# senli1073/SeisT

Hardware: NVIDIA H100
Metric: waveforms/sec (B,3,8192) seist_m_dpk fwd+bwd (higher is better)
Workload: dtype f32

## Files before the change

seist_b200/csrc/api.cu:

```cuda
#include <atomic>
#include <cstdio>
#include <cstdlib>
#include <cstring>
#include <vector>
#include "common.cuh"

namespace seist {

static thread_local char g_err[512] = "";
static std::atomic<uint64_t> g_launches{0};
static int g_sm_count = 0;

void set_error(const char* msg) {
  std::strncpy(g_err, msg, sizeof(g_err) - 1);
  g_err[sizeof(g_err) - 1] = 0;
}
void note_launch() { g_launches.fetch_add(1, std::memory_order_relaxed); }
int check_launch(const char* what) {
  cudaError_t e = cudaPeekAtLastError();
  if (e != cudaSuccess) {
    cudaGetLastError();
    std::snprintf(g_err, sizeof(g_err), "%s: %s", what, cudaGetErrorString(e));
    return (int)e;
  }
  return 0;
}

int launch_conv_fwd(const SeistOp& op, cudaStream_t s);
int launch_conv_bwd_data(const SeistOp& op, cudaStream_t s);
int launch_conv_bwd_w(const SeistOp& op, cudaStream_t s, int sm_count);
int launch_res_bwd(const SeistOp& op, cudaStream_t s);
int launch_att_fwd(const SeistOp& op, cudaStream_t s);
int launch_att_bwd_q(const SeistOp& op, cudaStream_t s);
int launch_att_bwd_kv(const SeistOp& op, cudaStream_t s);
int launch_headvec_fwd(const SeistOp& op, cudaStream_t s);
int launch_headvec_bwd(const SeistOp& op, cudaStream_t s);
int launch_bn_finalize(const SeistOp& op, bool fwd, cudaStream_t s);
bool pw_eligible(const SeistOp& op);
int launch_pw_fwd(const SeistOp& op, cudaStream_t s, int sm_count);
int launch_pw_bwd_data(const SeistOp& op, cudaStream_t s, int sm_count);
int launch_res_bwd4(const SeistOp& op, cudaStream_t s, int sm_count);
bool bww_eligible(const SeistOp& op);
int launch_bww_any(const SeistOp& op, cudaStream_t s, int sm_count);
bool convk_eligible(const SeistOp& op);
bool bwwk_eligible(const SeistOp& op);
int launch_grad_combine(const SeistOp& op, cudaStream_t s, int sm_count);
bool convk_bwd_data_eligible(const SeistOp& op);
int launch_bwwk(const SeistOp& op, cudaStream_t s, int sm_count);
int launch_convk_fwd(const SeistOp& op, cudaStream_t s);
int launch_convk_bwd_data(const SeistOp& op, cudaStream_t s);
int launch_bn_prepare(const SeistOp& op, bool fwd, cudaStream_t s);
int launch_stem_compose(const SeistOp& op, bool fwd, cudaStream_t s);
bool tcconv_eligible(const SeistOp& op, int mode);
int launch_tcconv(const SeistOp& op, int mode, cudaStream_t s, int sm_count);
int tcconv_error_flag();

int env_knob(const char* name, int def) {
  const char* e = std::getenv(name);
  return (e && *e) ? std::atoi(e) : def;
}
int bww_waves() {
  static int v = -1;
  if (v < 0) { const char* e = std::getenv("SEIST_BWW_WAVES"); v = (e && e[0] >= '1' && e[0] <= '4') ? e[0] - '0' : 2; }
  return v;
}
static int bwwk_mode() {
  static int v = -1;
  if (v < 0) { const char* e = std::getenv("SEIST_BWWK"); v = (e && e[0] == '0') ? 0 : 1; }
  return v;
}
static int tcc_mode() {
  static int v = -1;
  if (v < 0) { const char* e = std::getenv("SEIST_TCC"); v = !e ? 2 : (e[0] == '0' ? 0 : (e[0] == '1' ? 1 : 2)); }
  return v;
}
static bool tcc_auto(const SeistOp& op, int mode) {
  const int Kd = mode == 0 ? op.Cin : op.Cout;
  if (op.up_src_L > 0) return mode == 0 && Kd >= 32;
  if (op.k > 1) return mode == 0 ? (op.L_out <= 512 && Kd >= 16) : (op.L_out <= 256 && Kd >= 32);
  return mode == 0 && Kd >= 64 && op.L_out <= 256;
}
static bool use_tcc(const SeistOp& op, int mode) {
  const int m = tcc_mode();
  if (m == 0 || !tcconv_eligible(op, mode)) return false;
  return m == 1 || tcc_auto(op, mode);
}

static int sm_count() {
  if (g_sm_count == 0) {
    int dev = 0;
    cudaGetDevice(&dev);
    if (cudaDeviceGetAttribute(&g_sm_count, cudaDevAttrMultiProcessorCount, dev) != cudaSuccess || g_sm_count <= 0)
      g_sm_count = 132;
  }
  return g_sm_count;
}

static int validate_conv(const SeistOp& op) {
  if (op.groups <= 0 || op.Cin % op.groups || op.Cout % op.groups) { set_error("conv: channels not divisible by groups"); return -2; }
  if (op.k < 1 || op.stride < 1 || op.N < 1 || op.L_out < 1) { set_error("conv: bad geometry"); return -2; }
  if (op.n_in < 1 || op.n_in > SEIST_MAX_IN) { set_error("conv: bad n_in"); return -2; }
  if ((op.pool > 1 || op.up_src_L > 0) && op.n_in != 1) { set_error("conv: pool/upsample need a single input view"); return -2; }
  if (op.pool > 1 && (op.k != 1 || op.up_src_L > 0)) { set_error("conv: pool only with k=1"); return -2; }
  if (op.N > 65535) { set_error("conv: batch > 65535 per launch"); return -2; }
  return 0;
}

enum Family {
  F_NONE = 0, F_TCCONV_FWD, F_TCCONV_BWD_DATA, F_PW_FWD, F_CONVK_FWD, F_CONV_FWD, F_PW_BWD_DATA, F_CONVK_BWD_DATA,
  F_CONV_BWD_DATA, F_BWWK, F_BWW, F_CONV_BWD_W, F_RES_BWD, F_RES_BWD4, F_ATT_FWD, F_ATT_BWD_Q, F_ATT_BWD_KV, F_HEADVEC_FWD,
  F_HEADVEC_BWD, F_BN_FINALIZE_FWD, F_BN_FINALIZE_BWD, F_BN_PREPARE_FWD, F_BN_PREPARE_BWD, F_STEM_COMPOSE_FWD, F_STEM_COMPOSE_BWD,
  F_GRAD_COMBINE, F_ZERO
};
static const char* kFamilyName[] = {
  "none", "tcconv_fwd(wgmma+TMA)", "tcconv_bwd_data(wgmma+TMA)", "pw_fwd(simt)", "convk_fwd(simt)",
  "conv_fwd(simt)", "pw_bwd_data(simt)", "convk_bwd_data(simt)", "conv_bwd_data(simt)", "bwwk(simt)", "bww(simt)",
  "conv_bwd_w(simt)", "res_bwd", "res_bwd4", "att_fwd", "att_bwd_q", "att_bwd_kv", "headvec_fwd", "headvec_bwd", "bn_finalize_fwd",
  "bn_finalize_bwd", "bn_prepare_fwd", "bn_prepare_bwd", "stem_compose_fwd", "stem_compose_bwd", "grad_combine", "zero"
};

static Family choose(const SeistOp& op) {
  switch (op.kind) {
    case SEIST_OP_CONV_FWD:
      if (use_tcc(op, 0)) return F_TCCONV_FWD;
      if (pw_eligible(op)) return F_PW_FWD;
      return convk_eligible(op) ? F_CONVK_FWD : F_CONV_FWD;
    case SEIST_OP_CONV_BWD_DATA:
      if (use_tcc(op, 1)) return F_TCCONV_BWD_DATA;
      if (pw_eligible(op)) return F_PW_BWD_DATA;
      return convk_bwd_data_eligible(op) ? F_CONVK_BWD_DATA : F_CONV_BWD_DATA;
    case SEIST_OP_CONV_BWD_W:
      if (bwwk_mode() && bwwk_eligible(op)) return F_BWWK;
      return bww_eligible(op) ? F_BWW : F_CONV_BWD_W;
    case SEIST_OP_RES_BWD: return (op.L_out & 3) ? F_RES_BWD : F_RES_BWD4;
    case SEIST_OP_ATT_FWD: return F_ATT_FWD;
    case SEIST_OP_ATT_BWD_Q: return F_ATT_BWD_Q;
    case SEIST_OP_ATT_BWD_KV: return F_ATT_BWD_KV;
    case SEIST_OP_HEADVEC_FWD: return F_HEADVEC_FWD;
    case SEIST_OP_HEADVEC_BWD: return F_HEADVEC_BWD;
    case SEIST_OP_BN_FINALIZE_FWD: return F_BN_FINALIZE_FWD;
    case SEIST_OP_BN_FINALIZE_BWD: return F_BN_FINALIZE_BWD;
    case SEIST_OP_BN_PREPARE_FWD: return F_BN_PREPARE_FWD;
    case SEIST_OP_BN_PREPARE_BWD: return F_BN_PREPARE_BWD;
    case SEIST_OP_STEM_COMPOSE_FWD: return F_STEM_COMPOSE_FWD;
    case SEIST_OP_STEM_COMPOSE_BWD: return F_STEM_COMPOSE_BWD;
    case SEIST_OP_GRAD_COMBINE: return F_GRAD_COMBINE;
    case SEIST_OP_ZERO: return F_ZERO;
    default: return F_NONE;
  }
}

static int run_one(const SeistOp& op, cudaStream_t s) {
  if (op.kind == SEIST_OP_CONV_FWD || op.kind == SEIST_OP_CONV_BWD_DATA || op.kind == SEIST_OP_CONV_BWD_W) {
    int v = validate_conv(op);
    if (v) return v;
  }
  switch (choose(op)) {
    case F_TCCONV_FWD: return launch_tcconv(op, 0, s, sm_count());
    case F_TCCONV_BWD_DATA: return launch_tcconv(op, 1, s, sm_count());
    case F_PW_FWD: return launch_pw_fwd(op, s, sm_count());
    case F_CONVK_FWD: return launch_convk_fwd(op, s);
    case F_CONV_FWD: return launch_conv_fwd(op, s);
    case F_PW_BWD_DATA: return launch_pw_bwd_data(op, s, sm_count());
    case F_CONVK_BWD_DATA: return launch_convk_bwd_data(op, s);
    case F_CONV_BWD_DATA: return launch_conv_bwd_data(op, s);
    case F_BWWK: return launch_bwwk(op, s, sm_count());
    case F_BWW: return launch_bww_any(op, s, sm_count());
    case F_CONV_BWD_W: return launch_conv_bwd_w(op, s, sm_count());
    case F_RES_BWD: return launch_res_bwd(op, s);
    case F_RES_BWD4: return launch_res_bwd4(op, s, sm_count());
    case F_ATT_FWD: return launch_att_fwd(op, s);
    case F_ATT_BWD_Q: return launch_att_bwd_q(op, s);
    case F_ATT_BWD_KV: return launch_att_bwd_kv(op, s);
    case F_HEADVEC_FWD: return launch_headvec_fwd(op, s);
    case F_HEADVEC_BWD: return launch_headvec_bwd(op, s);
    case F_BN_FINALIZE_FWD: return launch_bn_finalize(op, true, s);
    case F_BN_FINALIZE_BWD: return launch_bn_finalize(op, false, s);
    case F_BN_PREPARE_FWD: return launch_bn_prepare(op, true, s);
    case F_BN_PREPARE_BWD: return launch_bn_prepare(op, false, s);
    case F_STEM_COMPOSE_FWD: return launch_stem_compose(op, true, s);
    case F_STEM_COMPOSE_BWD: return launch_stem_compose(op, false, s);
    case F_GRAD_COMBINE: return launch_grad_combine(op, s, sm_count());
    case F_ZERO: {
      cudaError_t e = cudaMemsetAsync(op.out.x, 0, op.zero_bytes, s);
      if (e != cudaSuccess) { set_error(cudaGetErrorString(e)); return (int)e; }
      return 0;
    }
    default: set_error("unknown op kind"); return -1;
  }
}

}

extern "C" {

int seist_plan_run(const SeistOp* ops, int32_t n, void* stream);
const char* seist_last_error(void);

int seist_abi_version(void) { return SEIST_ABI_VERSION; }
uint64_t seist_sizeof_op(void) { return sizeof(SeistOp); }
uint64_t seist_sizeof_bn(void) { return sizeof(SeistBN); }
const char* seist_last_error(void) { return seist::g_err; }
uint64_t seist_launch_count(void) { return seist::g_launches.load(); }
const char* seist_op_family(const SeistOp* op) { return op ? seist::kFamilyName[seist::choose(*op)] : "none"; }
int seist_tc_error_flag(void) { return seist::tcconv_error_flag(); }

static std::vector<cudaEvent_t> g_events[64];
static cudaEvent_t event_at(size_t i) {
  int dev = 0;
  cudaGetDevice(&dev);
  std::vector<cudaEvent_t>& pool = g_events[dev & 63];
  while (pool.size() <= i) {
    cudaEvent_t e = nullptr;
    if (cudaEventCreateWithFlags(&e, cudaEventDisableTiming) != cudaSuccess) return nullptr;
    pool.push_back(e);
  }
  return pool[i];
}
static int fork_join(cudaStream_t from, cudaStream_t to, size_t& ev) {
  cudaEvent_t e = event_at(ev++);
  if (e == nullptr) { seist::set_error("plan_run2: cudaEventCreate failed"); return (int)cudaErrorMemoryAllocation; }
  cudaError_t r = cudaEventRecord(e, from);
  if (r == cudaSuccess) r = cudaStreamWaitEvent(to, e, 0);
  if (r != cudaSuccess) { seist::set_error(cudaGetErrorString(r)); return (int)r; }
  return 0;
}

int seist_plan_run2(const SeistOp* ops, int32_t n, void* stream, void* side_stream) {
  if (side_stream == nullptr || side_stream == stream) return seist_plan_run(ops, n, stream);
  if (ops == nullptr || n < 0) { seist::set_error("plan_run2: bad arguments"); return -1; }
  cudaStream_t s = (cudaStream_t)stream, side = (cudaStream_t)side_stream;
  size_t ev = 0;
  bool forked = false, main_dirty = true;
  for (int i = 0; i < n; ++i) {
    const bool on_side = ops[i].kind == SEIST_OP_CONV_BWD_W || ops[i].kind == SEIST_OP_STEM_COMPOSE_BWD;
    int rc;
    if (on_side) {
      if (main_dirty) {
        const int fr = fork_join(s, side, ev);
        if (fr) return fr;
        main_dirty = false;
      }
      rc = seist::run_one(ops[i], side);
      forked = true;
    } else {
      rc = seist::run_one(ops[i], s);
      main_dirty = true;
    }
    if (rc != 0) {
      char buf[600];
      std::snprintf(buf, sizeof(buf), "op %d (kind %d): %s", i, ops[i].kind, seist::g_err);
      seist::set_error(buf);
      if (forked) fork_join(side, s, ev);
      return rc;
    }
  }
  if (forked) return fork_join(side, s, ev);
  return 0;
}

int seist_plan_run_lanes(const SeistOp* ops, int32_t n, void* const* streams, int32_t n_streams) {
  if (ops == nullptr || n < 0 || streams == nullptr || n_streams < 1 || n_streams > 8) { seist::set_error("plan_run_lanes: bad arguments"); return -1; }
  if (n_streams == 1) return seist_plan_run(ops, n, streams[0]);
  cudaStream_t s0 = (cudaStream_t)streams[0];
  size_t ev = (size_t)n;
  for (int l = 1; l < n_streams; ++l) {
    size_t e = ev;
    const int fr = fork_join(s0, (cudaStream_t)streams[l], e);
    if (fr) return fr;
  }
  int rc = 0;
  for (int i = 0; i < n && rc == 0; ++i) {
    const SeistOp& op = ops[i];
    const int lane = op.lane < 0 ? 0 : (op.lane >= n_streams ? n_streams - 1 : op.lane);
    cudaStream_t s = (cudaStream_t)streams[lane];
    for (int w = 0; w < op.n_wait && w < 4 && rc == 0; ++w) {
      if (op.wait_ev[w] < 0 || op.wait_ev[w] >= n) { seist::set_error("plan_run_lanes: bad event id"); rc = -1; break; }
      cudaEvent_t e = event_at((size_t)op.wait_ev[w]);
      cudaError_t r = e ? cudaStreamWaitEvent(s, e, 0) : cudaErrorMemoryAllocation;
      if (r != cudaSuccess) { seist::set_error(cudaGetErrorString(r)); rc = (int)r; }
    }
    if (rc) break;
    rc = seist::run_one(op, s);
    if (rc != 0) {
      char buf[600];
      std::snprintf(buf, sizeof(buf), "op %d (kind %d): %s", i, op.kind, seist_last_error());
      seist::set_error(buf);
      break;
    }
    if (op.rec_event >= 0) {
      cudaEvent_t e = op.rec_event < n ? event_at((size_t)op.rec_event) : nullptr;
      cudaError_t r = e ? cudaEventRecord(e, s) : cudaErrorMemoryAllocation;
      if (r != cudaSuccess) { seist::set_error(cudaGetErrorString(r)); rc = (int)r; }
    }
  }
  for (int l = 1; l < n_streams; ++l) {
    size_t e = (size_t)n + 1 + (size_t)l;
    const int jr = fork_join((cudaStream_t)streams[l], s0, e);
    if (jr && !rc) rc = jr;
  }
  return rc;
}

int seist_plan_run(const SeistOp* ops, int32_t n, void* stream) {
  if (ops == nullptr || n < 0) { seist::set_error("plan_run: bad arguments"); return -1; }
  cudaStream_t s = (cudaStream_t)stream;
  for (int i = 0; i < n; ++i) {
    int rc = seist::run_one(ops[i], s);
    if (rc != 0) {
      char buf[600];
      std::snprintf(buf, sizeof(buf), "op %d (kind %d): %s", i, ops[i].kind, seist::g_err);
      seist::set_error(buf);
      return rc;
    }
  }
  return 0;
}

}
```

seist_b200/csrc/tcconv.cu:

```cuda
#include <cuda.h>
#include <cstdlib>
#include <cstring>
#include "common.cuh"

namespace seist {

constexpr int TCC_EPI_WARPS = 8;
constexpr int TCC_XF_WARPS = 8;
constexpr int TCC_NT = 32 * (TCC_EPI_WARPS + TCC_XF_WARPS + 1);
constexpr int TCC_M = 128;
constexpr int TCC_MAX_STAGES = 8;
constexpr int TCC_NMAX = 128;
constexpr int TCC_ACC_PITCH = TCC_M + 4;

struct TccGeom {
  int mode;
  int Kd, Nd;
  int k, padl;
  int padA, toff;
  int src_len, dst_len;
  int KC, nchunks;
  int R, Rbox, Rp;
  int N_pad;
  int raw_stages, a_stages, b_resident;
  int n_raw;
  int raw_tensor_bytes;
  int a_part;
  int b_part;
  int a_stage;
  int has_dxd, has_bn, need_x;
  int up, up_S;
  int off_raw, off_a, off_b, off_tab_k, off_tab_n, off_red, off_acc, off_bar, smem_bytes;
};

struct TccMaps {
  CUtensorMap m[3];
};

struct TccK {
  float a, b, c;
  int view;
};
struct TccTgt {
  const float* x;
  float* g;
  long long nstride;
  float sc, sh, mu, istd;
  int act, bn, bnc, accum;
};

__device__ int g_tcc_err_dev = 0;

__device__ __forceinline__ uint32_t s32(const void* p) { return (uint32_t)__cvta_generic_to_shared(p); }

__device__ __forceinline__ uint64_t tcc_desc(uint32_t saddr, uint32_t lbo_bytes, uint32_t sbo_bytes) {
  uint64_t d = 0;
  d |= (uint64_t)((saddr >> 4) & 0x3FFFu);
  d |= (uint64_t)((lbo_bytes >> 4) & 0x3FFFu) << 16;
  d |= (uint64_t)((sbo_bytes >> 4) & 0x3FFFu) << 32;
  return d;
}
template <int N>
__device__ __forceinline__ void tcc_mma(float (&d)[N / 2], uint64_t adesc, uint64_t bdesc, uint32_t accum);
template <>
__device__ __forceinline__ void tcc_mma<32>(float (&d)[16], uint64_t adesc, uint64_t bdesc, uint32_t accum) {
  asm volatile(
      "{\n\t.reg .pred p;\n\tsetp.ne.b32 p, %18, 0;\n\t"
      "wgmma.mma_async.sync.aligned.m64n32k8.f32.tf32.tf32 {%0, %1, %2, %3, %4, %5, %6, %7, %8, %9, %10, %11, %12, %13, %14, %15}, %16, %17, p, 1, 1;\n\t}\n"
      : "+f"(d[0]), "+f"(d[1]), "+f"(d[2]), "+f"(d[3]), "+f"(d[4]), "+f"(d[5]), "+f"(d[6]), "+f"(d[7]), "+f"(d[8]), "+f"(d[9]), "+f"(d[10]), "+f"(d[11]), "+f"(d[12]), "+f"(d[13]), "+f"(d[14]), "+f"(d[15])
      : "l"(adesc), "l"(bdesc), "r"(accum));
}
template <>
__device__ __forceinline__ void tcc_mma<64>(float (&d)[32], uint64_t adesc, uint64_t bdesc, uint32_t accum) {
  asm volatile(
      "{\n\t.reg .pred p;\n\tsetp.ne.b32 p, %34, 0;\n\t"
      "wgmma.mma_async.sync.aligned.m64n64k8.f32.tf32.tf32 {%0, %1, %2, %3, %4, %5, %6, %7, %8, %9, %10, %11, %12, %13, %14, %15, %16, %17, %18, %19, %20, %21, %22, %23, %24, %25, %26, %27, %28, %29, %30, %31}, %32, %33, p, 1, 1;\n\t}\n"
      : "+f"(d[0]), "+f"(d[1]), "+f"(d[2]), "+f"(d[3]), "+f"(d[4]), "+f"(d[5]), "+f"(d[6]), "+f"(d[7]), "+f"(d[8]), "+f"(d[9]), "+f"(d[10]), "+f"(d[11]), "+f"(d[12]), "+f"(d[13]), "+f"(d[14]), "+f"(d[15]), "+f"(d[16]), "+f"(d[17]), "+f"(d[18]), "+f"(d[19]), "+f"(d[20]), "+f"(d[21]), "+f"(d[22]), "+f"(d[23]), "+f"(d[24]), "+f"(d[25]), "+f"(d[26]), "+f"(d[27]), "+f"(d[28]), "+f"(d[29]), "+f"(d[30]), "+f"(d[31])
      : "l"(adesc), "l"(bdesc), "r"(accum));
}
template <>
__device__ __forceinline__ void tcc_mma<128>(float (&d)[64], uint64_t adesc, uint64_t bdesc, uint32_t accum) {
  asm volatile(
      "{\n\t.reg .pred p;\n\tsetp.ne.b32 p, %66, 0;\n\t"
      "wgmma.mma_async.sync.aligned.m64n128k8.f32.tf32.tf32 {%0, %1, %2, %3, %4, %5, %6, %7, %8, %9, %10, %11, %12, %13, %14, %15, %16, %17, %18, %19, %20, %21, %22, %23, %24, %25, %26, %27, %28, %29, %30, %31, %32, %33, %34, %35, %36, %37, %38, %39, %40, %41, %42, %43, %44, %45, %46, %47, %48, %49, %50, %51, %52, %53, %54, %55, %56, %57, %58, %59, %60, %61, %62, %63}, %64, %65, p, 1, 1;\n\t}\n"
      : "+f"(d[0]), "+f"(d[1]), "+f"(d[2]), "+f"(d[3]), "+f"(d[4]), "+f"(d[5]), "+f"(d[6]), "+f"(d[7]), "+f"(d[8]), "+f"(d[9]), "+f"(d[10]), "+f"(d[11]), "+f"(d[12]), "+f"(d[13]), "+f"(d[14]), "+f"(d[15]), "+f"(d[16]), "+f"(d[17]), "+f"(d[18]), "+f"(d[19]), "+f"(d[20]), "+f"(d[21]), "+f"(d[22]), "+f"(d[23]), "+f"(d[24]), "+f"(d[25]), "+f"(d[26]), "+f"(d[27]), "+f"(d[28]), "+f"(d[29]), "+f"(d[30]), "+f"(d[31]), "+f"(d[32]), "+f"(d[33]), "+f"(d[34]), "+f"(d[35]), "+f"(d[36]), "+f"(d[37]), "+f"(d[38]), "+f"(d[39]), "+f"(d[40]), "+f"(d[41]), "+f"(d[42]), "+f"(d[43]), "+f"(d[44]), "+f"(d[45]), "+f"(d[46]), "+f"(d[47]), "+f"(d[48]), "+f"(d[49]), "+f"(d[50]), "+f"(d[51]), "+f"(d[52]), "+f"(d[53]), "+f"(d[54]), "+f"(d[55]), "+f"(d[56]), "+f"(d[57]), "+f"(d[58]), "+f"(d[59]), "+f"(d[60]), "+f"(d[61]), "+f"(d[62]), "+f"(d[63])
      : "l"(adesc), "l"(bdesc), "r"(accum));
}
template <int R>
__device__ __forceinline__ void tcc_keep(float (&d)[R]) {
#pragma unroll
  for (int i = 0; i < R; ++i) asm volatile("" : "+f"(d[i])::"memory");
}
__device__ __forceinline__ void tcc_arrive(uint32_t bar) {
  asm volatile("mbarrier.arrive.shared::cta.b64 _, [%0];" ::"r"(bar) : "memory");
}
__device__ __forceinline__ void tcc_expect_tx(uint32_t bar, uint32_t bytes) {
  asm volatile("mbarrier.arrive.expect_tx.shared::cta.b64 _, [%0], %1;" ::"r"(bar), "r"(bytes) : "memory");
}
__device__ __forceinline__ void tcc_tma3(uint32_t dst, const CUtensorMap* map, int c0, int c1, int c2, uint32_t bar) {
  asm volatile(
      "cp.async.bulk.tensor.3d.shared::cluster.global.tile.mbarrier::complete_tx::bytes [%0], [%1, {%2, %3, %4}], [%5];" ::"r"(dst),
      "l"((uint64_t)map), "r"(c0), "r"(c1), "r"(c2), "r"(bar)
      : "memory");
}
__device__ __forceinline__ bool tcc_wait(uint32_t bar, uint32_t parity, volatile int* abort_s) {
  uint32_t done = 0;
  for (int it = 0; it < (1 << 18); ++it) {
    asm volatile(
        "{\n\t.reg .pred p;\n\tmbarrier.try_wait.parity.shared::cta.b64 p, [%1], %2, %3;\n\tselp.b32 %0, 1, 0, p;\n\t}\n"
        : "=r"(done)
        : "r"(bar), "r"(parity), "r"(20000u)
        : "memory");
    if (done) return true;
    if ((it & 15) == 15 && *abort_s) return false;
  }
  *abort_s = 1;
  return false;
}
__device__ __forceinline__ void tcc_split(float x, float& hi, float& lo) {
  hi = __uint_as_float(__float_as_uint(x) & 0xFFFFE000u);
  lo = x - hi;
}
__device__ __forceinline__ float tcc_gelu(float x) { return gelu_f(x); }
__device__ __forceinline__ float tcc_gelu_grad(float x) { return gelu_grad_f(x); }

__device__ __forceinline__ float tcc_reduce16(float (&v)[16], int lane) {
#pragma unroll
  for (int half = 8, off = 16; half >= 1; half >>= 1, off >>= 1) {
    const bool up = (lane & off) != 0;
#pragma unroll
    for (int i = 0; i < 8; ++i) {
      if (i < half) {
        const float send = up ? v[i] : v[i + half];
        const float keep = up ? v[i + half] : v[i];
        v[i] = keep + __shfl_xor_sync(0xffffffffu, send, off);
      }
    }
  }
  return v[0] + __shfl_xor_sync(0xffffffffu, v[0], 1);
}
__device__ __forceinline__ int tcc_red_index(int lane) {
  return ((lane >> 4) & 1) * 8 + ((lane >> 3) & 1) * 4 + ((lane >> 2) & 1) * 2 + ((lane >> 1) & 1);
}

#define TCC_LD16(rr, col0)                                                                                               \
  _Pragma("unroll") for (int c_ = 0; c_ < 16; ++c_) rr[c_] = __float_as_uint(acc_s[((col0) + c_) * TCC_ACC_PITCH + srow]);

__device__ __forceinline__ int tcc_up_src0(int p0) { return ((p0 >> 1) - 1) & ~3; }

__device__ __forceinline__ float tcc_wval(const SeistOp& op, int mode, int t, int n, int c) {
  const int co = mode == 0 ? n : c, ci = mode == 0 ? c : n;
  const int tt = mode == 0 ? t : op.k - 1 - t;
  if (co >= op.Cout || ci >= op.Cin) return 0.f;
  const int cin_g = op.Cin / op.groups, cout_g = op.Cout / op.groups;
  const int g = co / cout_g;
  if (ci / cin_g != g) return 0.f;
  return __ldg(op.W + ((size_t)co * cin_g + (ci - g * cin_g)) * op.k + tt);
}

template <int MODE, bool F_GELU, bool F_ELEM, int NB>
__global__ void __launch_bounds__(TCC_NT, 1) tcconv_kernel(const __grid_constant__ SeistOp op, const __grid_constant__ TccGeom g,
                                                           const __grid_constant__ TccMaps maps) {
  extern __shared__ __align__(16) unsigned char tcc_raw[];
  unsigned char* base = tcc_raw + ((128u - (s32(tcc_raw) & 127u)) & 127u);
  unsigned char* raw_s = base + g.off_raw;
  unsigned char* a_s = base + g.off_a;
  unsigned char* b_s = base + g.off_b;
  TccK* tk_s = reinterpret_cast<TccK*>(base + g.off_tab_k);
  float* red_s = reinterpret_cast<float*>(base + g.off_red);
  uint64_t* bars = reinterpret_cast<uint64_t*>(base + g.off_bar);
  uint64_t* raw_full = bars;
  uint64_t* raw_empty = raw_full + TCC_MAX_STAGES;
  uint64_t* a_full = raw_empty + TCC_MAX_STAGES;
  uint64_t* a_empty = a_full + TCC_MAX_STAGES;
  volatile int* abort_s = reinterpret_cast<volatile int*>(a_empty + TCC_MAX_STAGES);
  float* acc_s = reinterpret_cast<float*>(base + g.off_acc);

  const int tid = threadIdx.x, lane = tid & 31;
  const int warp = __shfl_sync(0xffffffffu, tid >> 5, 0);
  const int Kd = g.Kd, Nd = g.Nd;
  const int Kd_pad = g.nchunks * g.KC;
  const int tiles_per_n = (g.dst_len + TCC_M - 1) / TCC_M;
  const int total = op.N * tiles_per_n;
  const bool has_bn_out = (op.out.bn >= 0 && op.out.g != nullptr);

  for (int c = tid; c < Kd_pad; c += TCC_NT) {
    TccK e;
    e.a = 0.f; e.b = 0.f; e.c = 0.f; e.view = 0;
    if (c < Kd) {
      if (MODE == 0) {
        int cv;
        const int vi = resolve_view(op, c, cv);
        view_coef(op, op.in[vi], cv, e.a, e.b);
        e.c = (float)op.in[vi].act;
        e.view = vi;
      } else {
        const OutGradCoef kc = out_grad_coef(op, c);
        e.a = kc.A; e.b = kc.Bx; e.c = kc.Cc;
      }
    }
    tk_s[c] = e;
  }
  if (MODE == 0) {
    float* ep_s = reinterpret_cast<float*>(base + g.off_tab_n);
    for (int co = tid; co < Nd; co += TCC_NT) {
      float b = 0.f, asc = 1.f, ash = 0.f, bsc = 1.f, bsh = 0.f;
      if (op.bias) b = op.bias[co];
      if (op.res_a.C > 0) view_coef(op, op.res_a, co, asc, ash);
      if (op.res_b.C > 0) view_coef(op, op.res_b, co, bsc, bsh);
      ep_s[co] = b;
      ep_s[Nd + co] = asc;
      ep_s[2 * Nd + co] = ash;
      ep_s[3 * Nd + co] = bsc;
      ep_s[4 * Nd + co] = bsh;
    }
  } else {
    TccTgt* tg_s = reinterpret_cast<TccTgt*>(base + g.off_tab_n);
    for (int ci = tid; ci < Nd; ci += TCC_NT) {
      int cv;
      const int vi = resolve_view(op, ci, cv);
      const SeistView& v = op.in[vi];
      TccTgt e;
      e.x = v.x + (size_t)(v.c0 + cv) * v.L;
      e.g = v.g ? v.g + (size_t)(v.c0 + cv) * v.L : nullptr;
      e.nstride = (long long)v.Ct * v.L;
      view_coef(op, v, cv, e.sc, e.sh);
      e.mu = 0.f; e.istd = 0.f;
      if (v.bn >= 0) view_khat(op, v, cv, e.mu, e.istd);
      e.act = v.act; e.bn = v.bn; e.bnc = v.bn_c0 + cv; e.accum = v.accum;
      tg_s[ci] = e;
    }
  }
  for (int i = tid; i < TCC_EPI_WARPS * 2 * Nd; i += TCC_NT) red_s[i] = 0.f;

  const int colpitchB = g.N_pad * 16;
  auto stage_b = [&](int chunk, unsigned char* b_hi, unsigned char* b_lo, int t0, int nthreads) {
    const int nq = g.KC >> 2;
    const int items = g.k * nq * g.N_pad;
    for (int idx = t0; idx < items; idx += nthreads) {
      const int n = idx % g.N_pad;
      const int rest = idx / g.N_pad;
      const int q = rest % nq, t = rest / nq;
      float4 hi, lo;
      float w[4];
#pragma unroll
      for (int j = 0; j < 4; ++j) {
        const int c = chunk * g.KC + 4 * q + j;
        w[j] = (n < Nd && c < Kd) ? tcc_wval(op, MODE, t, n, c) : 0.f;
      }
      tcc_split(w[0], hi.x, lo.x);
      tcc_split(w[1], hi.y, lo.y);
      tcc_split(w[2], hi.z, lo.z);
      tcc_split(w[3], hi.w, lo.w);
      const int off = (t * nq + q) * colpitchB + n * 16;
      *reinterpret_cast<float4*>(b_hi + off) = hi;
      *reinterpret_cast<float4*>(b_lo + off) = lo;
    }
  };
  if (g.b_resident)
    for (int ch = 0; ch < g.nchunks; ++ch) stage_b(ch, b_s + (size_t)ch * 2 * g.b_part, b_s + (size_t)ch * 2 * g.b_part + g.b_part, tid, TCC_NT);

  if (tid == 32) {
    for (int i = 0; i < TCC_MAX_STAGES; ++i) {
      asm volatile("mbarrier.init.shared::cta.b64 [%0], %1;" ::"r"(s32(&raw_full[i])), "r"(1) : "memory");
      asm volatile("mbarrier.init.shared::cta.b64 [%0], %1;" ::"r"(s32(&raw_empty[i])), "r"(TCC_XF_WARPS) : "memory");
      asm volatile("mbarrier.init.shared::cta.b64 [%0], %1;" ::"r"(s32(&a_full[i])), "r"(TCC_XF_WARPS) : "memory");
      asm volatile("mbarrier.init.shared::cta.b64 [%0], %1;" ::"r"(s32(&a_empty[i])), "r"(TCC_EPI_WARPS) : "memory");
    }
    *abort_s = 0;
    asm volatile("fence.mbarrier_init.release.cluster;" ::: "memory");
  }
  asm volatile("fence.proxy.async.shared::cta;" ::: "memory");
  __syncthreads();
  const uint64_t seed = load_seed(op.step_seed);

  if (warp == TCC_EPI_WARPS + TCC_XF_WARPS) {
    if (lane == 0) {
      int rs = 0;
      uint32_t rph = 0;
      const uint32_t stage_tx = (uint32_t)(g.n_raw * g.raw_tensor_bytes);
      const int nbox = g.KC >> 3;
      for (int tile = blockIdx.x; tile < total && !*abort_s; tile += gridDim.x) {
        const int n = tile / tiles_per_n;
        const int p0 = (tile - n * tiles_per_n) * TCC_M - g.padA;
        for (int ch = 0; ch < g.nchunks; ++ch) {
          if (!tcc_wait(s32(&raw_empty[rs]), rph ^ 1, abort_s)) break;
          const uint32_t bar = s32(&raw_full[rs]);
          tcc_expect_tx(bar, stage_tx);
          const uint32_t dst0 = s32(raw_s + (size_t)rs * g.n_raw * g.raw_tensor_bytes);
          for (int b = 0; b < nbox; ++b) {
            const int c = ch * g.KC + 8 * b;
            const uint32_t boxoff = (uint32_t)(8 * b * g.Rbox * 4);
            if (MODE == 0) {
              int cv = 0, vi = 0;
              if (c < Kd) vi = resolve_view(op, c, cv);
              else cv = 1 << 20;
              tcc_tma3(dst0 + boxoff, &maps.m[vi], g.up ? tcc_up_src0(p0) : p0, op.in[vi].c0 + cv, n, bar);
            } else {
              const int cc = c < Kd ? op.out.c0 + c : (1 << 20);
              int slot = 0;
              if (g.has_dxd) { tcc_tma3(dst0 + slot * g.raw_tensor_bytes + boxoff, &maps.m[0], p0, cc, n, bar); ++slot; }
              if (g.has_bn) { tcc_tma3(dst0 + slot * g.raw_tensor_bytes + boxoff, &maps.m[1], p0, cc, n, bar); ++slot; }
              if (g.need_x) { tcc_tma3(dst0 + slot * g.raw_tensor_bytes + boxoff, &maps.m[2], p0, cc, n, bar); ++slot; }
            }
          }
          if (++rs == g.raw_stages) { rs = 0; rph ^= 1; }
        }
      }
    }
  } else if (warp >= TCC_EPI_WARPS) {
    const int xw = warp - TCC_EPI_WARPS;
    int rs = 0, as = 0;
    uint32_t rph = 0, aph = 0;
    const int nq = g.KC >> 2, nrb = g.Rp >> 5;
    const int q = xw & (nq - 1);
    const int rb0 = xw / nq, rbs = TCC_XF_WARPS / nq;
    const int colpitchA = g.Rp * 16;
    const uint32_t thr = drop_threshold(op.p_elem);
    const float keep_s = op.p_elem > 0.f ? 1.0f / (1.0f - op.p_elem) : 1.f;
    const int raw_t = g.raw_tensor_bytes >> 2;
    for (int tile = blockIdx.x; tile < total && !*abort_s; tile += gridDim.x) {
      const int n = tile / tiles_per_n;
      const int p0 = (tile - n * tiles_per_n) * TCC_M - g.padA;
      float pfaf = 1.f;
      if (MODE == 1) pfaf = path_factor(op, seed, n) * alpha_factor(op, seed, n);
      for (int ch = 0; ch < g.nchunks; ++ch) {
        if (!tcc_wait(s32(&raw_full[rs]), rph, abort_s)) break;
        if (!tcc_wait(s32(&a_empty[as]), aph ^ 1, abort_s)) break;
        const float* raw = reinterpret_cast<const float*>(raw_s + (size_t)rs * g.n_raw * g.raw_tensor_bytes) + 4 * q * g.Rbox;
        unsigned char* a_hi = a_s + (size_t)as * g.a_stage + q * colpitchA;
        unsigned char* a_lo = a_hi + g.a_part;
        const int cbase = ch * g.KC + 4 * q;
        TccK e[4];
#pragma unroll
        for (int j = 0; j < 4; ++j) e[j] = tk_s[cbase + j];
        const int nvalid = Kd - cbase;
        for (int rb = rb0; rb < nrb; rb += 2 * rbs) {
          float t[2][4];
          int rrow[2];
          bool act[2];
#pragma unroll
          for (int h = 0; h < 2; ++h) {
            const int r = (rb + h * rbs) * 32 + lane;
            rrow[h] = r;
            act[h] = (rb + h * rbs) < nrb;
            const int p = p0 + r;
            const bool inb = act[h] && (r < g.R) && p >= 0 && p < g.src_len;
            const int rr = (act[h] && r < g.Rbox) ? r : 0;
            if (MODE == 0 && g.up) {
              const int pc = p < 0 ? 0 : p;
              const int i0 = pc == 0 ? 0 : (pc - 1) >> 1;
              const int i1 = min(i0 + 1, g.up_S - 1);
              const float w1 = pc == 0 ? 0.f : ((pc & 1) ? 0.25f : 0.75f);
              const int s0 = tcc_up_src0(p0);
              const int a0 = min(max(i0 - s0, 0), g.Rbox - 1), a1 = min(max(i1 - s0, 0), g.Rbox - 1);
#pragma unroll
              for (int j = 0; j < 4; ++j) {
                float f0 = fmaf(e[j].a, raw[j * g.Rbox + a0], e[j].b);
                float f1 = fmaf(e[j].a, raw[j * g.Rbox + a1], e[j].b);
                if (F_GELU && e[j].c != 0.f) { f0 = tcc_gelu(f0); f1 = tcc_gelu(f1); }
                const float v = fmaf(w1, f1 - f0, f0);
                t[h][j] = (inb && j < nvalid) ? v : 0.f;
              }
            } else if (MODE == 0) {
#pragma unroll
              for (int j = 0; j < 4; ++j) {
                float v = fmaf(e[j].a, raw[j * g.Rbox + rr], e[j].b);
                if (F_GELU && e[j].c != 0.f) v = tcc_gelu(v);
                t[h][j] = (inb && j < nvalid) ? v : 0.f;
              }
            } else {
              uint64_t hq = 0ull;
              if (F_ELEM) {
                const int ck = min(cbase + (lane & 3), Kd - 1);
                hq = rng_u64(seed, op.seed_elem, (((uint64_t)n * op.Cout + ck) * (uint64_t)op.L_out + (uint64_t)(inb ? p : 0)) >> 2);
              }
#pragma unroll
              for (int j = 0; j < 4; ++j) {
                const int ro = j * g.Rbox + rr;
                int slot = 0;
                float dxd = 0.f, du = 0.f, x = 0.f;
                if (g.has_dxd) { dxd = raw[ro]; ++slot; }
                if (g.has_bn) { du = raw[slot * raw_t + ro]; ++slot; }
                if (g.need_x) { x = raw[slot * raw_t + ro]; }
                float gv = dxd + fmaf(e[j].a, du, fmaf(e[j].b, x, e[j].c));
                if (op.out_act == SEIST_OUT_SIGMOID) gv *= x * (1.f - x);
                gv *= pfaf;
                if (F_ELEM) {
                  const uint64_t hh = __shfl_sync(0xffffffffu, hq, (lane & ~3) | j);
                  gv *= (((uint32_t)(hh >> (16 * (p & 3))) & 0xFFFFu) >= thr) ? keep_s : 0.f;
                }
                t[h][j] = (inb && j < nvalid) ? gv : 0.f;
              }
            }
          }
#pragma unroll
          for (int h = 0; h < 2; ++h) {
            if (!act[h]) continue;
            float4 hi, lo;
            tcc_split(t[h][0], hi.x, lo.x);
            tcc_split(t[h][1], hi.y, lo.y);
            tcc_split(t[h][2], hi.z, lo.z);
            tcc_split(t[h][3], hi.w, lo.w);
            *reinterpret_cast<float4*>(a_hi + rrow[h] * 16) = hi;
            *reinterpret_cast<float4*>(a_lo + rrow[h] * 16) = lo;
          }
        }
        if (!g.b_resident) {
          unsigned char* bst = a_s + (size_t)as * g.a_stage + 2 * g.a_part;
          stage_b(ch, bst, bst + g.b_part, xw * 32 + lane, TCC_XF_WARPS * 32);
        }
        asm volatile("fence.proxy.async.shared::cta;" ::: "memory");
        __syncwarp();
        if (lane == 0) {
          tcc_arrive(s32(&a_full[as]));
          tcc_arrive(s32(&raw_empty[rs]));
        }
        if (++rs == g.raw_stages) { rs = 0; rph ^= 1; }
        if (++as == g.a_stages) { as = 0; aph ^= 1; }
      }
    }
  } else {
    const int eg = warp >> 2, wq = warp & 3;
    const int L = g.dst_len;
    const bool stats = MODE == 0 ? ((op.out.bn >= 0) && op.bn_table[op.out.bn >= 0 ? op.out.bn : 0].use_batch) : true;
    const float* ep_s = reinterpret_cast<const float*>(base + g.off_tab_n);
    const TccTgt* tg_s = reinterpret_cast<const TccTgt*>(base + g.off_tab_n);
    const uint32_t thr = drop_threshold(op.p_elem);
    const float keep_s = op.p_elem > 0.f ? 1.0f / (1.0f - op.p_elem) : 1.f;
    float* my_red = red_s + warp * 2 * Nd;
    const bool has_ra = MODE == 0 && op.res_a.C > 0, has_rb = MODE == 0 && op.res_b.C > 0;
    const bool sig = op.out_act == SEIST_OUT_SIGMOID;
    const size_t Ls = (size_t)L;
    const uint32_t colpitchA = (uint32_t)g.Rp * 16u;
    const int nq = g.KC >> 2;
    const int srow = 32 * wq + lane;
    int as = 0;
    uint32_t aph = 0;
    for (int tile = blockIdx.x; tile < total; tile += gridDim.x) {
      float acc[NB / 2];
      bool run = true;
      int prev = -1;
      for (int ch = 0; ch < g.nchunks; ++ch) {
        run = run && tcc_wait(s32(&a_full[as]), aph, abort_s);
        {
          const uint32_t a_hi = s32(a_s + (size_t)as * g.a_stage) + (uint32_t)(eg * 64 * 16);
          const uint32_t a_lo = a_hi + (uint32_t)g.a_part;
          uint32_t b_hi;
          if (g.b_resident) b_hi = s32(b_s + (size_t)ch * 2 * g.b_part);
          else b_hi = s32(a_s + (size_t)as * g.a_stage) + 2u * (uint32_t)g.a_part;
          const uint32_t b_lo = b_hi + (uint32_t)g.b_part;
          const int ksteps = min(g.KC, Kd - ch * g.KC + 7) >> 3;
          asm volatile("wgmma.fence.sync.aligned;" ::: "memory");
          for (int t = 0; t < g.k; ++t) {
            for (int j = 0; j < ksteps; ++j) {
              const uint32_t aoff = (uint32_t)(2 * j) * colpitchA + (uint32_t)(t + g.toff) * 16u;
              const uint32_t boff = (uint32_t)(t * nq + 2 * j) * (uint32_t)colpitchB;
              const uint64_t ah = tcc_desc(a_hi + aoff, colpitchA, 128), al = tcc_desc(a_lo + aoff, colpitchA, 128);
              const uint64_t bh = tcc_desc(b_hi + boff, (uint32_t)colpitchB, 128), bl = tcc_desc(b_lo + boff, (uint32_t)colpitchB, 128);
              tcc_mma<NB>(acc, ah, bh, (ch > 0 || t > 0 || j > 0) ? 1u : 0u);
              tcc_mma<NB>(acc, al, bh, 1u);
              tcc_mma<NB>(acc, ah, bl, 1u);
            }
          }
          asm volatile("wgmma.commit_group.sync.aligned;" ::: "memory");
          asm volatile("wgmma.wait_group.sync.aligned 1;" ::: "memory");
        }
        if (prev >= 0) {
          __syncwarp();
          if (lane == 0) tcc_arrive(s32(&a_empty[prev]));
        }
        prev = as;
        if (++as == g.a_stages) { as = 0; aph ^= 1; }
      }
      asm volatile("wgmma.wait_group.sync.aligned 0;" ::: "memory");
      tcc_keep(acc);
      __syncwarp();
      if (lane == 0) tcc_arrive(s32(&a_empty[prev]));
      asm volatile("bar.sync 1, 256;" ::: "memory");
      if (run) {
        const int r0 = eg * 64 + wq * 16 + (lane >> 2);
        const int cl = 2 * (lane & 3);
#pragma unroll
        for (int e = 0; e < NB / 2; ++e)
          acc_s[(8 * (e >> 2) + cl + (e & 1)) * TCC_ACC_PITCH + r0 + 8 * ((e >> 1) & 1)] = acc[e];
      }
      asm volatile("bar.sync 1, 256;" ::: "memory");
      if (!run || *abort_s) continue;
      const int n = tile / tiles_per_n;
      const int l = (tile - n * tiles_per_n) * TCC_M + srow;
      const bool ok = l < L;
      const int ls = ok ? l : 0;
      if (MODE == 0) {
        const float pf = path_factor(op, seed, n), af = alpha_factor(op, seed, n);
        float* optr = op.out.x + ((size_t)n * op.out.Ct + op.out.c0 + 16 * eg) * Ls + ls;
        const float* ra = has_ra ? op.res_a.x + ((size_t)n * op.res_a.Ct + op.res_a.c0 + 16 * eg) * Ls + ls : nullptr;
        const float* rb = has_rb ? op.res_b.x + ((size_t)n * op.res_b.Ct + op.res_b.c0 + 16 * eg) * Ls + ls : nullptr;
#pragma unroll 1
        for (int c0 = 16 * eg; c0 < Nd; c0 += 32) {
          uint32_t rr[16];
          TCC_LD16(rr, c0);
          const int nv = min(16, Nd - c0);
          float val[16];
#pragma unroll
          for (int c = 0; c < 16; ++c) val[c] = (__uint_as_float(rr[c]) + ep_s[min(c0 + c, Nd - 1)]) * pf;
          if (F_ELEM) {
#pragma unroll
            for (int qd = 0; qd < 4; ++qd) {
              const int ck = min(c0 + 4 * qd + (lane & 3), Nd - 1);
              const uint64_t hq = rng_u64(seed, op.seed_elem, (((uint64_t)n * Nd + ck) * (uint64_t)L + (uint64_t)ls) >> 2);
#pragma unroll
              for (int j = 0; j < 4; ++j) {
                const uint64_t hh = __shfl_sync(0xffffffffu, hq, (lane & ~3) | j);
                val[4 * qd + j] *= ((uint32_t)(hh >> (16 * (l & 3))) & 0xFFFFu) >= thr ? keep_s : 0.f;
              }
            }
          }
          if (has_ra) {
            float rv[16];
#pragma unroll
            for (int c = 0; c < 16; ++c) rv[c] = __ldg(ra + (size_t)min(c, nv - 1) * Ls);
#pragma unroll
            for (int c = 0; c < 16; ++c) val[c] += fmaf(ep_s[Nd + min(c0 + c, Nd - 1)], rv[c], ep_s[2 * Nd + min(c0 + c, Nd - 1)]);
            ra += 32 * Ls;
          }
          if (af != 1.f) {
#pragma unroll
            for (int c = 0; c < 16; ++c) val[c] *= af;
          }
          if (has_rb) {
            float rv[16];
#pragma unroll
            for (int c = 0; c < 16; ++c) rv[c] = __ldg(rb + (size_t)min(c, nv - 1) * Ls);
#pragma unroll
            for (int c = 0; c < 16; ++c) val[c] += fmaf(ep_s[3 * Nd + min(c0 + c, Nd - 1)], rv[c], ep_s[4 * Nd + min(c0 + c, Nd - 1)]);
            rb += 32 * Ls;
          }
          if (sig) {
#pragma unroll
            for (int c = 0; c < 16; ++c) val[c] = sigmoid_f(val[c]);
          }
          float* op_c = optr;
#pragma unroll
          for (int c = 0; c < 16; ++c) {
            const bool w = ok && c < nv;
            if (w) *op_c = val[c];
            val[c] = w ? val[c] : 0.f;
            op_c += Ls;
          }
          optr += 32 * Ls;
          if (stats) {
            float s2[16];
#pragma unroll
            for (int c = 0; c < 16; ++c) s2[c] = val[c] * val[c];
            const float t1 = tcc_reduce16(val, lane), t2 = tcc_reduce16(s2, lane);
            const int co = c0 + tcc_red_index(lane);
            if ((lane & 1) == 0 && co < Nd) {
              my_red[2 * co] += t1;
              my_red[2 * co + 1] += t2;
            }
          }
        }
      } else {
#pragma unroll 1
        for (int c0 = 16 * eg; c0 < Nd; c0 += 32) {
          uint32_t rr[16];
          TCC_LD16(rr, c0);
          float xv[16], ov[16];
#pragma unroll
          for (int c = 0; c < 16; ++c) {
            const TccTgt& e = tg_s[min(c0 + c, Nd - 1)];
            const bool live = ok && (c0 + c < Nd) && e.g != nullptr;
            const long long off = (long long)n * e.nstride + ls;
            xv[c] = (live && (e.bn >= 0 || (F_GELU && e.act == SEIST_ACT_GELU))) ? __ldg(e.x + off) : 0.f;
            ov[c] = (live && e.accum) ? e.g[off] : 0.f;
          }
          float s1[16], s2[16];
#pragma unroll
          for (int c = 0; c < 16; ++c) {
            const TccTgt& e = tg_s[min(c0 + c, Nd - 1)];
            const bool live = ok && (c0 + c < Nd) && e.g != nullptr;
            float gg = live ? __uint_as_float(rr[c]) : 0.f;
            if (F_GELU && e.act == SEIST_ACT_GELU) gg *= tcc_gelu_grad(fmaf(e.sc, xv[c], e.sh));
            const bool st = live && e.bn >= 0;
            s1[c] = st ? gg : 0.f;
            s2[c] = st ? gg * ((xv[c] - e.mu) * e.istd) : 0.f;
            if (live) e.g[(long long)n * e.nstride + l] = gg + ov[c];
          }
          const float t1 = tcc_reduce16(s1, lane), t2 = tcc_reduce16(s2, lane);
          const int ci = c0 + tcc_red_index(lane);
          if ((lane & 1) == 0 && ci < Nd) {
            my_red[2 * ci] += t1;
            my_red[2 * ci + 1] += t2;
          }
        }
      }
    }
  }

  __syncthreads();
  if (MODE == 0) {
    const bool stats = (op.out.bn >= 0) && op.bn_table[op.out.bn >= 0 ? op.out.bn : 0].use_batch;
    if (stats) {
      const SeistBN& e = op.bn_table[op.out.bn];
      for (int i = tid; i < 2 * Nd; i += TCC_NT) {
        float s = 0.f;
        for (int w = 0; w < TCC_EPI_WARPS; ++w) s += red_s[w * 2 * Nd + i];
        atomicAdd(&e.stat_acc[(i & 1) * e.C + op.out.bn_c0 + (i >> 1)], (double)s);
      }
    }
  } else {
    const TccTgt* tg_s = reinterpret_cast<const TccTgt*>(base + g.off_tab_n);
    for (int i = tid; i < 2 * Nd; i += TCC_NT) {
      const TccTgt& t = tg_s[i >> 1];
      if (t.g != nullptr && t.bn >= 0) {
        float s = 0.f;
        for (int w = 0; w < TCC_EPI_WARPS; ++w) s += red_s[w * 2 * Nd + i];
        const SeistBN& e = op.bn_table[t.bn];
        atomicAdd(&e.gstat_acc[(i & 1) * e.C + t.bnc], (double)s);
      }
    }
  }
  if (tid == 0 && *abort_s) atomicExch(&g_tcc_err_dev, 1);
}

typedef CUresult (*EncodeTiledFn)(CUtensorMap*, CUtensorMapDataType, cuuint32_t, void*, const cuuint64_t*, const cuuint64_t*,
                                  const cuuint32_t*, const cuuint32_t*, CUtensorMapInterleave, CUtensorMapSwizzle,
                                  CUtensorMapL2promotion, CUtensorMapFloatOOBfill);
static EncodeTiledFn tcc_encode_fn() {
  static EncodeTiledFn fn = nullptr;
  static bool tried = false;
  if (!tried) {
    tried = true;
    void* p = nullptr;
    cudaDriverEntryPointQueryResult qres;
    if (cudaGetDriverEntryPoint("cuTensorMapEncodeTiled", &p, cudaEnableDefault, &qres) == cudaSuccess &&
        qres == cudaDriverEntryPointSuccess)
      fn = reinterpret_cast<EncodeTiledFn>(p);
  }
  return fn;
}

static int tcc_make_map(CUtensorMap* m, const float* basep, int L, int Ct, int N, int box_rows) {
  EncodeTiledFn fn = tcc_encode_fn();
  if (!fn) { set_error("tcconv: cuTensorMapEncodeTiled unavailable"); return -3; }
  const cuuint64_t dims[3] = {(cuuint64_t)L, (cuuint64_t)Ct, (cuuint64_t)N};
  const cuuint64_t strides[2] = {(cuuint64_t)L * 4ull, (cuuint64_t)L * (cuuint64_t)Ct * 4ull};
  const cuuint32_t box[3] = {(cuuint32_t)box_rows, 8u, 1u};
  const cuuint32_t estr[3] = {1u, 1u, 1u};
  CUresult r = fn(m, CU_TENSOR_MAP_DATA_TYPE_FLOAT32, 3, const_cast<float*>(basep), dims, strides, box, estr,
                  CU_TENSOR_MAP_INTERLEAVE_NONE, CU_TENSOR_MAP_SWIZZLE_NONE, CU_TENSOR_MAP_L2_PROMOTION_L2_128B,
                  CU_TENSOR_MAP_FLOAT_OOB_FILL_NONE);
  if (r != CUDA_SUCCESS) { set_error("tcconv: cuTensorMapEncodeTiled failed"); return -3; }
  return 0;
}


bool tcconv_eligible(const SeistOp& op, int mode) {
  if (op.stride != 1 || op.pool > 1 || op.k > 32) return false;
  if ((mode == 0 ? op.Cout : op.Cin) > TCC_NMAX) return false;
  if (op.L_in != op.L_out || (op.L_out & 3)) return false;
  if (op.up_src_L > 0) {
    if (mode != 0 || op.n_in != 1 || op.L_in != 2 * op.up_src_L || (op.up_src_L & 3) || op.in[0].L != op.up_src_L) return false;
    return (reinterpret_cast<uintptr_t>(op.in[0].x) & 15) == 0;
  }
  if (op.Cout > 256 || op.Cin > 256) return false;
  if (op.k > 1 && op.p_elem > 0.f) return false;
  for (int i = 0; i < op.n_in; ++i) {
    if (op.in[i].L != op.L_in) return false;
    if (op.n_in > 1 && (op.in[i].C & 7)) return false;
    if ((reinterpret_cast<uintptr_t>(op.in[i].x) & 15) != 0) return false;
  }
  if (mode == 1) {
    bool any = false;
    for (int i = 0; i < op.n_in; ++i) any = any || op.in[i].g != nullptr;
    if (!any) return false;
    if ((reinterpret_cast<uintptr_t>(op.out.x) & 15) != 0) return false;
  }
  return true;
}

static bool tcc_geometry(const SeistOp& op, int mode, TccGeom& g) {
  g = TccGeom{};
  g.mode = mode;
  g.Kd = mode == 0 ? op.Cin : op.Cout;
  g.Nd = mode == 0 ? op.Cout : op.Cin;
  g.k = op.k;
  g.padl = mode == 0 ? op.pad_left : op.k - 1 - op.pad_left;
  g.src_len = mode == 0 ? op.L_in : op.L_out;
  g.dst_len = mode == 0 ? op.L_out : op.L_in;
  g.padA = (g.padl + 3) & ~3;
  g.toff = g.padA - g.padl;
  g.R = TCC_M + op.k - 1 + g.toff;
  g.up = (mode == 0 && op.up_src_L > 0) ? 1 : 0;
  g.up_S = op.up_src_L;
  g.Rbox = g.up ? ((g.R / 2 + 6 + 3) & ~3) : ((g.R + 3) & ~3);
  g.Rp = (g.R + 31) & ~31;
  g.N_pad = g.Nd <= 32 ? 32 : (g.Nd <= 64 ? 64 : 128);
  if (g.N_pad > TCC_NMAX) return false;
  const bool has_bn = (op.out.bn >= 0 && op.out.g != nullptr);
  g.has_dxd = (mode == 1 && op.out_dxd != nullptr) ? 1 : 0;
  g.has_bn = (mode == 1 && has_bn) ? 1 : 0;
  g.need_x = (mode == 1 && (has_bn || op.out_act == SEIST_OUT_SIGMOID)) ? 1 : 0;
  g.n_raw = mode == 0 ? 1 : g.has_dxd + g.has_bn + g.need_x;
  if (g.n_raw == 0) return false;
  const int tab_n = mode == 0 ? 5 * g.Nd * 4 : g.Nd * (int)sizeof(TccTgt);
  const int budget = 220 * 1024;
  int kcs[3] = {32, 16, 8};
  {
    const int k8 = (g.Kd + 7) & ~7;
    auto waste = [&](int kc) { return ((k8 + kc - 1) / kc) * kc - k8; };
    for (int i = 0; i < 3; ++i)
      for (int j = i + 1; j < 3; ++j)
        if (waste(kcs[j]) < waste(kcs[i])) { const int tmp = kcs[i]; kcs[i] = kcs[j]; kcs[j] = tmp; }
  }
  for (int resident = 1; resident >= 0; --resident) {
    for (int ki = 0; ki < 3; ++ki) {
      const int KC = kcs[ki];
      g.KC = KC;
      g.nchunks = (g.Kd + KC - 1) / KC;
      g.raw_tensor_bytes = KC * g.Rbox * 4;
      g.a_part = (KC / 4) * g.Rp * 16;
      g.b_part = g.k * (KC / 4) * g.N_pad * 16;
      g.b_resident = resident;
      const int b_bytes = resident ? g.nchunks * 2 * g.b_part : 0;
      const int a_stage = 2 * g.a_part + (resident ? 0 : 2 * g.b_part);
      g.a_stage = a_stage;
      const int raw_stage = g.n_raw * g.raw_tensor_bytes;
      const int acc_bytes = g.N_pad * TCC_ACC_PITCH * 4;
      const int fixed = b_bytes + g.nchunks * KC * (int)sizeof(TccK) + tab_n + 16 * g.Nd * 4 + acc_bytes + 4 * TCC_MAX_STAGES * 8 + 64 + 256;
      for (int st = 4; st >= 2; --st) {
        const int rst = st + 1 > TCC_MAX_STAGES ? TCC_MAX_STAGES : st + 1;
        const int tot = fixed + st * a_stage + rst * raw_stage;
        if (tot <= budget) {
          g.a_stages = st;
          g.raw_stages = rst;
          int off = 0;
          g.off_raw = off; off += rst * raw_stage;
          g.off_a = off; off += st * a_stage;
          g.off_b = off; off += b_bytes;
          g.off_tab_k = off; off += g.nchunks * KC * (int)sizeof(TccK);
          off = (off + 15) & ~15;
          g.off_tab_n = off; off += tab_n;
          off = (off + 15) & ~15;
          g.off_red = off; off += 16 * g.Nd * 4;
          off = (off + 15) & ~15;
          g.off_acc = off; off += acc_bytes;
          g.off_bar = off; off += 4 * TCC_MAX_STAGES * 8 + 64;
          g.smem_bytes = off + 128;
          return true;
        }
      }
    }
  }
  return false;
}

template <int MODE, bool G, bool E, int NB>
static int tcc_go_nb(const SeistOp& op, const TccGeom& g, const TccMaps& maps, unsigned grid, cudaStream_t s) {
  static bool attr_set[64] = {false};
  int dev = 0;
  cudaGetDevice(&dev);
  if (!attr_set[dev & 63]) {
    cudaError_t e = cudaFuncSetAttribute(tcconv_kernel<MODE, G, E, NB>, cudaFuncAttributeMaxDynamicSharedMemorySize, 227 * 1024);
    if (e != cudaSuccess) { set_error(cudaGetErrorString(e)); return (int)e; }
    attr_set[dev & 63] = true;
  }
  tcconv_kernel<MODE, G, E, NB><<<grid, TCC_NT, g.smem_bytes, s>>>(op, g, maps);
  return 0;
}
template <int MODE, bool G, bool E>
static int tcc_go(const SeistOp& op, const TccGeom& g, const TccMaps& maps, unsigned grid, cudaStream_t s) {
  if (g.N_pad == 32) return tcc_go_nb<MODE, G, E, 32>(op, g, maps, grid, s);
  if (g.N_pad == 64) return tcc_go_nb<MODE, G, E, 64>(op, g, maps, grid, s);
  return tcc_go_nb<MODE, G, E, 128>(op, g, maps, grid, s);
}

int launch_tcconv(const SeistOp& op, int mode, cudaStream_t s, int sm_count) {
  TccGeom g;
  if (!tcc_geometry(op, mode, g)) { set_error("tcconv: no shared-memory configuration"); return -2; }
  TccMaps maps;
  std::memset(&maps, 0, sizeof(maps));
  int rc = 0;
  if (mode == 0) {
    for (int i = 0; i < op.n_in && !rc; ++i) rc = tcc_make_map(&maps.m[i], op.in[i].x, op.in[i].L, op.in[i].Ct, op.N, g.Rbox);
  } else {
    if (g.has_dxd) rc = tcc_make_map(&maps.m[0], op.out_dxd, op.out.L, op.out.Ct, op.N, g.Rbox);
    if (!rc && g.has_bn) rc = tcc_make_map(&maps.m[1], op.out.g, op.out.L, op.out.Ct, op.N, g.Rbox);
    if (!rc && g.need_x) rc = tcc_make_map(&maps.m[2], op.out.x, op.out.L, op.out.Ct, op.N, g.Rbox);
  }
  if (rc) return rc;
  const long tiles = (long)op.N * ((g.dst_len + TCC_M - 1) / TCC_M);
  long gr = sm_count;
  if (gr > tiles) gr = tiles;
  const unsigned grid = (unsigned)(gr < 1 ? 1 : gr);
  bool gelu = false;
  for (int i = 0; i < op.n_in; ++i) gelu = gelu || op.in[i].act == SEIST_ACT_GELU;
  const bool elem = op.p_elem > 0.f;
  if (mode == 0) {
    if (gelu) rc = elem ? tcc_go<0, true, true>(op, g, maps, grid, s) : tcc_go<0, true, false>(op, g, maps, grid, s);
    else rc = elem ? tcc_go<0, false, true>(op, g, maps, grid, s) : tcc_go<0, false, false>(op, g, maps, grid, s);
  } else {
    if (gelu) rc = elem ? tcc_go<1, true, true>(op, g, maps, grid, s) : tcc_go<1, true, false>(op, g, maps, grid, s);
    else rc = elem ? tcc_go<1, false, true>(op, g, maps, grid, s) : tcc_go<1, false, false>(op, g, maps, grid, s);
  }
  if (rc) return rc;
  note_launch();
  return check_launch(mode == 0 ? "tcconv_fwd" : "tcconv_bwd_data");
}

int tcconv_error_flag() {
  int v = 0;
  cudaMemcpyFromSymbol(&v, g_tcc_err_dev, sizeof(int));
  return v;
}

}
```

Before: 9270.

## Add TMA+wgmma tensor-core weight-gradient kernel for pointwise convolutions

Adds a new warp-specialized weight-gradient kernel for k=1 convolutions. Producer warps load output gradients and inputs with TMA, apply the BN/activation gradient transform and split values into TF32 hi/lo panels. Consumer warps then accumulate dW with wgmma m64nN, using three products for near-FP32 accuracy, and flush with atomics. It is enabled by default ahead of the SIMT bww path, and shared wgmma/TMA helpers move into a common header. The cost is the 3x MMA split, atomic contention on dW across persistent CTAs, and a new pipeline that could hang or abort.

```diff
diff --git a/seist_b200/csrc/api.cu b/seist_b200/csrc/api.cu
--- a/seist_b200/csrc/api.cu
+++ b/seist_b200/csrc/api.cu
@@ -54,6 +54,9 @@
 bool tcconv_eligible(const SeistOp& op, int mode);
 int launch_tcconv(const SeistOp& op, int mode, cudaStream_t s, int sm_count);
 int tcconv_error_flag();
+bool tcwgrad_eligible(const SeistOp& op);
+int launch_tcwgrad(const SeistOp& op, cudaStream_t s, int ctas);
+int tcwgrad_error_flag();
 
 int env_knob(const char* name, int def) {
   const char* e = std::getenv(name);
@@ -84,6 +87,12 @@
   const int m = tcc_mode();
   if (m == 0 || !tcconv_eligible(op, mode)) return false;
   return m == 1 || tcc_auto(op, mode);
+}
+
+static bool use_tcw(const SeistOp& op) {
+  static int v = -1;
+  if (v < 0) { const char* e = std::getenv("SEIST_TCW"); v = (e && e[0] == '0') ? 0 : 1; }
+  return v && tcwgrad_eligible(op);
 }
 
 static int sm_count() {
@@ -108,13 +117,13 @@
 
 enum Family {
   F_NONE = 0, F_TCCONV_FWD, F_TCCONV_BWD_DATA, F_PW_FWD, F_CONVK_FWD, F_CONV_FWD, F_PW_BWD_DATA, F_CONVK_BWD_DATA,
-  F_CONV_BWD_DATA, F_BWWK, F_BWW, F_CONV_BWD_W, F_RES_BWD, F_RES_BWD4, F_ATT_FWD, F_ATT_BWD_Q, F_ATT_BWD_KV, F_HEADVEC_FWD,
+  F_CONV_BWD_DATA, F_BWWK, F_TCWGRAD, F_BWW, F_CONV_BWD_W, F_RES_BWD, F_RES_BWD4, F_ATT_FWD, F_ATT_BWD_Q, F_ATT_BWD_KV, F_HEADVEC_FWD,
   F_HEADVEC_BWD, F_BN_FINALIZE_FWD, F_BN_FINALIZE_BWD, F_BN_PREPARE_FWD, F_BN_PREPARE_BWD, F_STEM_COMPOSE_FWD, F_STEM_COMPOSE_BWD,
   F_GRAD_COMBINE, F_ZERO
 };
 static const char* kFamilyName[] = {
   "none", "tcconv_fwd(wgmma+TMA)", "tcconv_bwd_data(wgmma+TMA)", "pw_fwd(simt)", "convk_fwd(simt)",
-  "conv_fwd(simt)", "pw_bwd_data(simt)", "convk_bwd_data(simt)", "conv_bwd_data(simt)", "bwwk(simt)", "bww(simt)",
+  "conv_fwd(simt)", "pw_bwd_data(simt)", "convk_bwd_data(simt)", "conv_bwd_data(simt)", "bwwk(simt)", "tcwgrad(wgmma+TMA)", "bww(simt)",
   "conv_bwd_w(simt)", "res_bwd", "res_bwd4", "att_fwd", "att_bwd_q", "att_bwd_kv", "headvec_fwd", "headvec_bwd", "bn_finalize_fwd",
   "bn_finalize_bwd", "bn_prepare_fwd", "bn_prepare_bwd", "stem_compose_fwd", "stem_compose_bwd", "grad_combine", "zero"
 };
@@ -131,6 +140,7 @@
       return convk_bwd_data_eligible(op) ? F_CONVK_BWD_DATA : F_CONV_BWD_DATA;
     case SEIST_OP_CONV_BWD_W:
       if (bwwk_mode() && bwwk_eligible(op)) return F_BWWK;
+      if (use_tcw(op)) return F_TCWGRAD;
       return bww_eligible(op) ? F_BWW : F_CONV_BWD_W;
     case SEIST_OP_RES_BWD: return (op.L_out & 3) ? F_RES_BWD : F_RES_BWD4;
     case SEIST_OP_ATT_FWD: return F_ATT_FWD;
@@ -165,6 +175,7 @@
     case F_CONVK_BWD_DATA: return launch_convk_bwd_data(op, s);
     case F_CONV_BWD_DATA: return launch_conv_bwd_data(op, s);
     case F_BWWK: return launch_bwwk(op, s, sm_count());
+    case F_TCWGRAD: return launch_tcwgrad(op, s, env_knob("SEIST_TCW_CTAS", 2 * sm_count()));
     case F_BWW: return launch_bww_any(op, s, sm_count());
     case F_CONV_BWD_W: return launch_conv_bwd_w(op, s, sm_count());
     case F_RES_BWD: return launch_res_bwd(op, s);
@@ -203,7 +214,7 @@
 const char* seist_last_error(void) { return seist::g_err; }
 uint64_t seist_launch_count(void) { return seist::g_launches.load(); }
 const char* seist_op_family(const SeistOp* op) { return op ? seist::kFamilyName[seist::choose(*op)] : "none"; }
-int seist_tc_error_flag(void) { return seist::tcconv_error_flag(); }
+int seist_tc_error_flag(void) { return seist::tcconv_error_flag() | seist::tcwgrad_error_flag(); }
 
 static std::vector<cudaEvent_t> g_events[64];
 static cudaEvent_t event_at(size_t i) {
diff --git a/seist_b200/csrc/tc_common.cuh b/seist_b200/csrc/tc_common.cuh
--- /dev/null
+++ b/seist_b200/csrc/tc_common.cuh
@@ -0,0 +1,98 @@
+#pragma once
+#include <cuda.h>
+#include "common.cuh"
+
+namespace seist {
+
+__device__ __forceinline__ uint32_t s32(const void* p) { return (uint32_t)__cvta_generic_to_shared(p); }
+
+__device__ __forceinline__ uint64_t tcc_desc(uint32_t saddr, uint32_t lbo_bytes, uint32_t sbo_bytes) {
+  uint64_t d = 0;
+  d |= (uint64_t)((saddr >> 4) & 0x3FFFu);
+  d |= (uint64_t)((lbo_bytes >> 4) & 0x3FFFu) << 16;
+  d |= (uint64_t)((sbo_bytes >> 4) & 0x3FFFu) << 32;
+  return d;
+}
+template <int N>
+__device__ __forceinline__ void tcc_mma(float (&d)[N / 2], uint64_t adesc, uint64_t bdesc, uint32_t accum);
+template <>
+__device__ __forceinline__ void tcc_mma<16>(float (&d)[8], uint64_t adesc, uint64_t bdesc, uint32_t accum) {
+  asm volatile(
+      "{\n\t.reg .pred p;\n\tsetp.ne.b32 p, %10, 0;\n\t"
+      "wgmma.mma_async.sync.aligned.m64n16k8.f32.tf32.tf32 {%0, %1, %2, %3, %4, %5, %6, %7}, %8, %9, p, 1, 1;\n\t}\n"
+      : "+f"(d[0]), "+f"(d[1]), "+f"(d[2]), "+f"(d[3]), "+f"(d[4]), "+f"(d[5]), "+f"(d[6]), "+f"(d[7])
+      : "l"(adesc), "l"(bdesc), "r"(accum));
+}
+template <>
+__device__ __forceinline__ void tcc_mma<32>(float (&d)[16], uint64_t adesc, uint64_t bdesc, uint32_t accum) {
+  asm volatile(
+      "{\n\t.reg .pred p;\n\tsetp.ne.b32 p, %18, 0;\n\t"
+      "wgmma.mma_async.sync.aligned.m64n32k8.f32.tf32.tf32 {%0, %1, %2, %3, %4, %5, %6, %7, %8, %9, %10, %11, %12, %13, %14, %15}, %16, %17, p, 1, 1;\n\t}\n"
+      : "+f"(d[0]), "+f"(d[1]), "+f"(d[2]), "+f"(d[3]), "+f"(d[4]), "+f"(d[5]), "+f"(d[6]), "+f"(d[7]), "+f"(d[8]), "+f"(d[9]), "+f"(d[10]), "+f"(d[11]), "+f"(d[12]), "+f"(d[13]), "+f"(d[14]), "+f"(d[15])
+      : "l"(adesc), "l"(bdesc), "r"(accum));
+}
+template <>
+__device__ __forceinline__ void tcc_mma<64>(float (&d)[32], uint64_t adesc, uint64_t bdesc, uint32_t accum) {
+  asm volatile(
+      "{\n\t.reg .pred p;\n\tsetp.ne.b32 p, %34, 0;\n\t"
+      "wgmma.mma_async.sync.aligned.m64n64k8.f32.tf32.tf32 {%0, %1, %2, %3, %4, %5, %6, %7, %8, %9, %10, %11, %12, %13, %14, %15, %16, %17, %18, %19, %20, %21, %22, %23, %24, %25, %26, %27, %28, %29, %30, %31}, %32, %33, p, 1, 1;\n\t}\n"
+      : "+f"(d[0]), "+f"(d[1]), "+f"(d[2]), "+f"(d[3]), "+f"(d[4]), "+f"(d[5]), "+f"(d[6]), "+f"(d[7]), "+f"(d[8]), "+f"(d[9]), "+f"(d[10]), "+f"(d[11]), "+f"(d[12]), "+f"(d[13]), "+f"(d[14]), "+f"(d[15]), "+f"(d[16]), "+f"(d[17]), "+f"(d[18]), "+f"(d[19]), "+f"(d[20]), "+f"(d[21]), "+f"(d[22]), "+f"(d[23]), "+f"(d[24]), "+f"(d[25]), "+f"(d[26]), "+f"(d[27]), "+f"(d[28]), "+f"(d[29]), "+f"(d[30]), "+f"(d[31])
+      : "l"(adesc), "l"(bdesc), "r"(accum));
+}
+template <>
+__device__ __forceinline__ void tcc_mma<128>(float (&d)[64], uint64_t adesc, uint64_t bdesc, uint32_t accum) {
+  asm volatile(
+      "{\n\t.reg .pred p;\n\tsetp.ne.b32 p, %66, 0;\n\t"
+      "wgmma.mma_async.sync.aligned.m64n128k8.f32.tf32.tf32 {%0, %1, %2, %3, %4, %5, %6, %7, %8, %9, %10, %11, %12, %13, %14, %15, %16, %17, %18, %19, %20, %21, %22, %23, %24, %25, %26, %27, %28, %29, %30, %31, %32, %33, %34, %35, %36, %37, %38, %39, %40, %41, %42, %43, %44, %45, %46, %47, %48, %49, %50, %51, %52, %53, %54, %55, %56, %57, %58, %59, %60, %61, %62, %63}, %64, %65, p, 1, 1;\n\t}\n"
+      : "+f"(d[0]), "+f"(d[1]), "+f"(d[2]), "+f"(d[3]), "+f"(d[4]), "+f"(d[5]), "+f"(d[6]), "+f"(d[7]), "+f"(d[8]), "+f"(d[9]), "+f"(d[10]), "+f"(d[11]), "+f"(d[12]), "+f"(d[13]), "+f"(d[14]), "+f"(d[15]), "+f"(d[16]), "+f"(d[17]), "+f"(d[18]), "+f"(d[19]), "+f"(d[20]), "+f"(d[21]), "+f"(d[22]), "+f"(d[23]), "+f"(d[24]), "+f"(d[25]), "+f"(d[26]), "+f"(d[27]), "+f"(d[28]), "+f"(d[29]), "+f"(d[30]), "+f"(d[31]), "+f"(d[32]), "+f"(d[33]), "+f"(d[34]), "+f"(d[35]), "+f"(d[36]), "+f"(d[37]), "+f"(d[38]), "+f"(d[39]), "+f"(d[40]), "+f"(d[41]), "+f"(d[42]), "+f"(d[43]), "+f"(d[44]), "+f"(d[45]), "+f"(d[46]), "+f"(d[47]), "+f"(d[48]), "+f"(d[49]), "+f"(d[50]), "+f"(d[51]), "+f"(d[52]), "+f"(d[53]), "+f"(d[54]), "+f"(d[55]), "+f"(d[56]), "+f"(d[57]), "+f"(d[58]), "+f"(d[59]), "+f"(d[60]), "+f"(d[61]), "+f"(d[62]), "+f"(d[63])
+      : "l"(adesc), "l"(bdesc), "r"(accum));
+}
+template <int R>
+__device__ __forceinline__ void tcc_keep(float (&d)[R]) {
+#pragma unroll
+  for (int i = 0; i < R; ++i) asm volatile("" : "+f"(d[i])::"memory");
+}
+__device__ __forceinline__ void tcc_arrive(uint32_t bar) {
+  asm volatile("mbarrier.arrive.shared::cta.b64 _, [%0];" ::"r"(bar) : "memory");
+}
+__device__ __forceinline__ void tcc_expect_tx(uint32_t bar, uint32_t bytes) {
+  asm volatile("mbarrier.arrive.expect_tx.shared::cta.b64 _, [%0], %1;" ::"r"(bar), "r"(bytes) : "memory");
+}
+__device__ __forceinline__ void tcc_tma3(uint32_t dst, const CUtensorMap* map, int c0, int c1, int c2, uint32_t bar) {
+  asm volatile(
+      "cp.async.bulk.tensor.3d.shared::cluster.global.tile.mbarrier::complete_tx::bytes [%0], [%1, {%2, %3, %4}], [%5];" ::"r"(dst),
+      "l"((uint64_t)map), "r"(c0), "r"(c1), "r"(c2), "r"(bar)
+      : "memory");
+}
+__device__ __forceinline__ bool tcc_wait(uint32_t bar, uint32_t parity, volatile int* abort_s) {
+  uint32_t done = 0;
+  for (int it = 0; it < (1 << 18); ++it) {
+    asm volatile(
+        "{\n\t.reg .pred p;\n\tmbarrier.try_wait.parity.shared::cta.b64 p, [%1], %2, %3;\n\tselp.b32 %0, 1, 0, p;\n\t}\n"
+        : "=r"(done)
+        : "r"(bar), "r"(parity), "r"(20000u)
+        : "memory");
+    if (done) return true;
+    if ((it & 15) == 15 && *abort_s) return false;
+  }
+  *abort_s = 1;
+  return false;
+}
+__device__ __forceinline__ void tcc_split(float x, float& hi, float& lo) {
+  hi = __uint_as_float(__float_as_uint(x) & 0xFFFFE000u);
+  lo = x - hi;
+}
+
+__device__ __forceinline__ float tc_conv_input(float raw, float sc, float sh, bool gelu) {
+  const float v = fmaf(sc, raw, sh);
+  return gelu ? gelu_f(v) : v;
+}
+__device__ __forceinline__ float tc_out_grad(float dxd, float du, float x, float A, float Bx, float Cc, bool sig, float pfaf) {
+  float gv = dxd + fmaf(A, du, fmaf(Bx, x, Cc));
+  if (sig) gv *= x * (1.f - x);
+  return gv * pfaf;
+}
+
+int tcc_make_map(CUtensorMap* m, const float* basep, int L, int Ct, int N, int box_rows);
+
+}
diff --git a/seist_b200/csrc/tcconv.cu b/seist_b200/csrc/tcconv.cu
--- a/seist_b200/csrc/tcconv.cu
+++ b/seist_b200/csrc/tcconv.cu
@@ -1,7 +1,7 @@
 #include <cuda.h>
 #include <cstdlib>
 #include <cstring>
-#include "common.cuh"
+#include "tc_common.cuh"
 
 namespace seist {
 
@@ -51,77 +51,6 @@
 
 __device__ int g_tcc_err_dev = 0;
 
-__device__ __forceinline__ uint32_t s32(const void* p) { return (uint32_t)__cvta_generic_to_shared(p); }
-
-__device__ __forceinline__ uint64_t tcc_desc(uint32_t saddr, uint32_t lbo_bytes, uint32_t sbo_bytes) {
-  uint64_t d = 0;
-  d |= (uint64_t)((saddr >> 4) & 0x3FFFu);
-  d |= (uint64_t)((lbo_bytes >> 4) & 0x3FFFu) << 16;
-  d |= (uint64_t)((sbo_bytes >> 4) & 0x3FFFu) << 32;
-  return d;
-}
-template <int N>
-__device__ __forceinline__ void tcc_mma(float (&d)[N / 2], uint64_t adesc, uint64_t bdesc, uint32_t accum);
-template <>
-__device__ __forceinline__ void tcc_mma<32>(float (&d)[16], uint64_t adesc, uint64_t bdesc, uint32_t accum) {
-  asm volatile(
-      "{\n\t.reg .pred p;\n\tsetp.ne.b32 p, %18, 0;\n\t"
-      "wgmma.mma_async.sync.aligned.m64n32k8.f32.tf32.tf32 {%0, %1, %2, %3, %4, %5, %6, %7, %8, %9, %10, %11, %12, %13, %14, %15}, %16, %17, p, 1, 1;\n\t}\n"
-      : "+f"(d[0]), "+f"(d[1]), "+f"(d[2]), "+f"(d[3]), "+f"(d[4]), "+f"(d[5]), "+f"(d[6]), "+f"(d[7]), "+f"(d[8]), "+f"(d[9]), "+f"(d[10]), "+f"(d[11]), "+f"(d[12]), "+f"(d[13]), "+f"(d[14]), "+f"(d[15])
-      : "l"(adesc), "l"(bdesc), "r"(accum));
-}
-template <>
-__device__ __forceinline__ void tcc_mma<64>(float (&d)[32], uint64_t adesc, uint64_t bdesc, uint32_t accum) {
-  asm volatile(
-      "{\n\t.reg .pred p;\n\tsetp.ne.b32 p, %34, 0;\n\t"
-      "wgmma.mma_async.sync.aligned.m64n64k8.f32.tf32.tf32 {%0, %1, %2, %3, %4, %5, %6, %7, %8, %9, %10, %11, %12, %13, %14, %15, %16, %17, %18, %19, %20, %21, %22, %23, %24, %25, %26, %27, %28, %29, %30, %31}, %32, %33, p, 1, 1;\n\t}\n"
-      : "+f"(d[0]), "+f"(d[1]), "+f"(d[2]), "+f"(d[3]), "+f"(d[4]), "+f"(d[5]), "+f"(d[6]), "+f"(d[7]), "+f"(d[8]), "+f"(d[9]), "+f"(d[10]), "+f"(d[11]), "+f"(d[12]), "+f"(d[13]), "+f"(d[14]), "+f"(d[15]), "+f"(d[16]), "+f"(d[17]), "+f"(d[18]), "+f"(d[19]), "+f"(d[20]), "+f"(d[21]), "+f"(d[22]), "+f"(d[23]), "+f"(d[24]), "+f"(d[25]), "+f"(d[26]), "+f"(d[27]), "+f"(d[28]), "+f"(d[29]), "+f"(d[30]), "+f"(d[31])
-      : "l"(adesc), "l"(bdesc), "r"(accum));
-}
-template <>
-__device__ __forceinline__ void tcc_mma<128>(float (&d)[64], uint64_t adesc, uint64_t bdesc, uint32_t accum) {
-  asm volatile(
-      "{\n\t.reg .pred p;\n\tsetp.ne.b32 p, %66, 0;\n\t"
-      "wgmma.mma_async.sync.aligned.m64n128k8.f32.tf32.tf32 {%0, %1, %2, %3, %4, %5, %6, %7, %8, %9, %10, %11, %12, %13, %14, %15, %16, %17, %18, %19, %20, %21, %22, %23, %24, %25, %26, %27, %28, %29, %30, %31, %32, %33, %34, %35, %36, %37, %38, %39, %40, %41, %42, %43, %44, %45, %46, %47, %48, %49, %50, %51, %52, %53, %54, %55, %56, %57, %58, %59, %60, %61, %62, %63}, %64, %65, p, 1, 1;\n\t}\n"
-      : "+f"(d[0]), "+f"(d[1]), "+f"(d[2]), "+f"(d[3]), "+f"(d[4]), "+f"(d[5]), "+f"(d[6]), "+f"(d[7]), "+f"(d[8]), "+f"(d[9]), "+f"(d[10]), "+f"(d[11]), "+f"(d[12]), "+f"(d[13]), "+f"(d[14]), "+f"(d[15]), "+f"(d[16]), "+f"(d[17]), "+f"(d[18]), "+f"(d[19]), "+f"(d[20]), "+f"(d[21]), "+f"(d[22]), "+f"(d[23]), "+f"(d[24]), "+f"(d[25]), "+f"(d[26]), "+f"(d[27]), "+f"(d[28]), "+f"(d[29]), "+f"(d[30]), "+f"(d[31]), "+f"(d[32]), "+f"(d[33]), "+f"(d[34]), "+f"(d[35]), "+f"(d[36]), "+f"(d[37]), "+f"(d[38]), "+f"(d[39]), "+f"(d[40]), "+f"(d[41]), "+f"(d[42]), "+f"(d[43]), "+f"(d[44]), "+f"(d[45]), "+f"(d[46]), "+f"(d[47]), "+f"(d[48]), "+f"(d[49]), "+f"(d[50]), "+f"(d[51]), "+f"(d[52]), "+f"(d[53]), "+f"(d[54]), "+f"(d[55]), "+f"(d[56]), "+f"(d[57]), "+f"(d[58]), "+f"(d[59]), "+f"(d[60]), "+f"(d[61]), "+f"(d[62]), "+f"(d[63])
-      : "l"(adesc), "l"(bdesc), "r"(accum));
-}
-template <int R>
-__device__ __forceinline__ void tcc_keep(float (&d)[R]) {
-#pragma unroll
-  for (int i = 0; i < R; ++i) asm volatile("" : "+f"(d[i])::"memory");
-}
-__device__ __forceinline__ void tcc_arrive(uint32_t bar) {
-  asm volatile("mbarrier.arrive.shared::cta.b64 _, [%0];" ::"r"(bar) : "memory");
-}
-__device__ __forceinline__ void tcc_expect_tx(uint32_t bar, uint32_t bytes) {
-  asm volatile("mbarrier.arrive.expect_tx.shared::cta.b64 _, [%0], %1;" ::"r"(bar), "r"(bytes) : "memory");
-}
-__device__ __forceinline__ void tcc_tma3(uint32_t dst, const CUtensorMap* map, int c0, int c1, int c2, uint32_t bar) {
-  asm volatile(
-      "cp.async.bulk.tensor.3d.shared::cluster.global.tile.mbarrier::complete_tx::bytes [%0], [%1, {%2, %3, %4}], [%5];" ::"r"(dst),
-      "l"((uint64_t)map), "r"(c0), "r"(c1), "r"(c2), "r"(bar)
-      : "memory");
-}
-__device__ __forceinline__ bool tcc_wait(uint32_t bar, uint32_t parity, volatile int* abort_s) {
-  uint32_t done = 0;
-  for (int it = 0; it < (1 << 18); ++it) {
-    asm volatile(
-        "{\n\t.reg .pred p;\n\tmbarrier.try_wait.parity.shared::cta.b64 p, [%1], %2, %3;\n\tselp.b32 %0, 1, 0, p;\n\t}\n"
-        : "=r"(done)
-        : "r"(bar), "r"(parity), "r"(20000u)
-        : "memory");
-    if (done) return true;
-    if ((it & 15) == 15 && *abort_s) return false;
-  }
-  *abort_s = 1;
-  return false;
-}
-__device__ __forceinline__ void tcc_split(float x, float& hi, float& lo) {
-  hi = __uint_as_float(__float_as_uint(x) & 0xFFFFE000u);
-  lo = x - hi;
-}
-__device__ __forceinline__ float tcc_gelu(float x) { return gelu_f(x); }
 __device__ __forceinline__ float tcc_gelu_grad(float x) { return gelu_grad_f(x); }
 
 __device__ __forceinline__ float tcc_reduce16(float (&v)[16], int lane) {
@@ -356,17 +285,16 @@
               const int a0 = min(max(i0 - s0, 0), g.Rbox - 1), a1 = min(max(i1 - s0, 0), g.Rbox - 1);
 #pragma unroll
               for (int j = 0; j < 4; ++j) {
-                float f0 = fmaf(e[j].a, raw[j * g.Rbox + a0], e[j].b);
-                float f1 = fmaf(e[j].a, raw[j * g.Rbox + a1], e[j].b);
-                if (F_GELU && e[j].c != 0.f) { f0 = tcc_gelu(f0); f1 = tcc_gelu(f1); }
+                const bool gl = F_GELU && e[j].c != 0.f;
+                const float f0 = tc_conv_input(raw[j * g.Rbox + a0], e[j].a, e[j].b, gl);
+                const float f1 = tc_conv_input(raw[j * g.Rbox + a1], e[j].a, e[j].b, gl);
                 const float v = fmaf(w1, f1 - f0, f0);
                 t[h][j] = (inb && j < nvalid) ? v : 0.f;
               }
             } else if (MODE == 0) {
 #pragma unroll
               for (int j = 0; j < 4; ++j) {
-                float v = fmaf(e[j].a, raw[j * g.Rbox + rr], e[j].b);
-                if (F_GELU && e[j].c != 0.f) v = tcc_gelu(v);
+                const float v = tc_conv_input(raw[j * g.Rbox + rr], e[j].a, e[j].b, F_GELU && e[j].c != 0.f);
                 t[h][j] = (inb && j < nvalid) ? v : 0.f;
               }
             } else {
@@ -383,9 +311,7 @@
                 if (g.has_dxd) { dxd = raw[ro]; ++slot; }
                 if (g.has_bn) { du = raw[slot * raw_t + ro]; ++slot; }
                 if (g.need_x) { x = raw[slot * raw_t + ro]; }
-                float gv = dxd + fmaf(e[j].a, du, fmaf(e[j].b, x, e[j].c));
-                if (op.out_act == SEIST_OUT_SIGMOID) gv *= x * (1.f - x);
-                gv *= pfaf;
+                float gv = tc_out_grad(dxd, du, x, e[j].a, e[j].b, e[j].c, op.out_act == SEIST_OUT_SIGMOID, pfaf);
                 if (F_ELEM) {
                   const uint64_t hh = __shfl_sync(0xffffffffu, hq, (lane & ~3) | j);
                   gv *= (((uint32_t)(hh >> (16 * (p & 3))) & 0xFFFFu) >= thr) ? keep_s : 0.f;
@@ -641,7 +567,7 @@
   return fn;
 }
 
-static int tcc_make_map(CUtensorMap* m, const float* basep, int L, int Ct, int N, int box_rows) {
+int tcc_make_map(CUtensorMap* m, const float* basep, int L, int Ct, int N, int box_rows) {
   EncodeTiledFn fn = tcc_encode_fn();
   if (!fn) { set_error("tcconv: cuTensorMapEncodeTiled unavailable"); return -3; }
   const cuuint64_t dims[3] = {(cuuint64_t)L, (cuuint64_t)Ct, (cuuint64_t)N};
diff --git a/seist_b200/csrc/tcwgrad.cu b/seist_b200/csrc/tcwgrad.cu
--- /dev/null
+++ b/seist_b200/csrc/tcwgrad.cu
@@ -0,0 +1,407 @@
+#include <cstring>
+#include "tc_common.cuh"
+
+namespace seist {
+
+constexpr int TCW_XF_WARPS = 7;
+constexpr int TCW_NT = 32 * (4 + TCW_XF_WARPS + 1);
+constexpr int TCW_MAX_STAGES = 8;
+constexpr int TCW_MAX_P_STAGES = 4;
+constexpr int TCW_SMEM_BUDGET = 100 * 1024;
+constexpr int TCW_PANEL_SLACK = 1024;
+
+struct TcwGeom {
+  int S;
+  int QI;
+  int g0, gC, x0, xC;
+  int split_g, blk;
+  int ng, has_dxd, has_bn, need_x;
+  int g_pitch, x_pitch;
+  int g_is_a;
+  int raw_stages, raw_stage, raw_g;
+  int part_a, part_b;
+  int p_stage, p_stages;
+  int off_raw, off_p, off_tab_g, off_tab_x, off_db, off_bar, smem_bytes;
+};
+struct TcwMaps {
+  CUtensorMap g[3];
+  CUtensorMap x[SEIST_MAX_IN];
+};
+
+__device__ int g_tcw_err_dev = 0;
+
+template <int NB, int MT>
+__global__ void __launch_bounds__(TCW_NT, 1) tcwgrad_kernel(const __grid_constant__ SeistOp op, const __grid_constant__ TcwGeom g,
+                                                            const __grid_constant__ TcwMaps maps) {
+  extern __shared__ __align__(16) unsigned char tcw_raw[];
+  unsigned char* base = tcw_raw + ((128u - (s32(tcw_raw) & 127u)) & 127u);
+  unsigned char* raw_s = base + g.off_raw;
+  unsigned char* p_s = base + g.off_p;
+  float4* tg_s = reinterpret_cast<float4*>(base + g.off_tab_g);
+  float4* tx_s = reinterpret_cast<float4*>(base + g.off_tab_x);
+  float* db_s = reinterpret_cast<float*>(base + g.off_db);
+  uint64_t* raw_full = reinterpret_cast<uint64_t*>(base + g.off_bar);
+  uint64_t* raw_empty = raw_full + TCW_MAX_STAGES;
+  uint64_t* p_full = raw_empty + TCW_MAX_STAGES;
+  uint64_t* p_empty = p_full + TCW_MAX_STAGES;
+  volatile int* abort_s = reinterpret_cast<volatile int*>(p_empty + TCW_MAX_STAGES);
+
+  const int tid = threadIdx.x, lane = tid & 31;
+  const int warp = __shfl_sync(0xffffffffu, tid >> 5, 0);
+  const int g0 = g.split_g ? g.g0 + blockIdx.y * g.blk : g.g0;
+  const int x0 = g.split_g ? g.x0 : g.x0 + blockIdx.y * g.blk;
+  const int gC = g.split_g ? min(g.blk, op.Cout - g0) : g.gC;
+  const int xC = g.split_g ? g.xC : min(g.blk, op.Cin - x0);
+  const int gO = (gC + 7) >> 3, xO = (xC + 7) >> 3;
+  const int L = op.L_out;
+  const int tiles_per_n = (L + g.S - 1) / g.S;
+  const int total = op.N * tiles_per_n;
+
+  for (int c = tid; c < 8 * gO; c += TCW_NT) {
+    float4 e = make_float4(0.f, 0.f, 0.f, 0.f);
+    if (c < gC) {
+      const OutGradCoef k = out_grad_coef(op, g0 + c);
+      e = make_float4(k.A, k.Bx, k.Cc, 0.f);
+    }
+    tg_s[c] = e;
+    db_s[c] = 0.f;
+  }
+  for (int c = tid; c < 8 * xO; c += TCW_NT) {
+    float4 e = make_float4(1.f, 0.f, 0.f, 0.f);
+    if (c < xC) {
+      int cv;
+      const int vi = resolve_view(op, x0 + c, cv);
+      view_coef(op, op.in[vi], cv, e.x, e.y);
+      e.z = op.in[vi].act == SEIST_ACT_GELU ? 1.f : 0.f;
+    }
+    tx_s[c] = e;
+  }
+  if (tid == 32) {
+    for (int i = 0; i < TCW_MAX_STAGES; ++i) {
+      asm volatile("mbarrier.init.shared::cta.b64 [%0], %1;" ::"r"(s32(&raw_full[i])), "r"(1) : "memory");
+      asm volatile("mbarrier.init.shared::cta.b64 [%0], %1;" ::"r"(s32(&raw_empty[i])), "r"(TCW_XF_WARPS) : "memory");
+      asm volatile("mbarrier.init.shared::cta.b64 [%0], %1;" ::"r"(s32(&p_full[i])), "r"(TCW_XF_WARPS) : "memory");
+      asm volatile("mbarrier.init.shared::cta.b64 [%0], %1;" ::"r"(s32(&p_empty[i])), "r"(4) : "memory");
+    }
+    *abort_s = 0;
+    asm volatile("fence.mbarrier_init.release.cluster;" ::: "memory");
+  }
+  __syncthreads();
+  const uint64_t seed = load_seed(op.step_seed);
+
+  if (warp == 4 + TCW_XF_WARPS) {
+    if (lane == 0) {
+      int rs = 0;
+      uint32_t rph = 0;
+      const int box = 8 * g.S * 4;
+      for (int tile = blockIdx.x; tile < total && !*abort_s; tile += gridDim.x) {
+        const int n = tile / tiles_per_n;
+        const int l0 = (tile - n * tiles_per_n) * g.S;
+        if (!tcc_wait(s32(&raw_empty[rs]), rph ^ 1, abort_s)) break;
+        const uint32_t bar = s32(&raw_full[rs]);
+        tcc_expect_tx(bar, (uint32_t)((g.ng * gO + xO) * box));
+        const uint32_t dst = s32(raw_s + (size_t)rs * g.raw_stage);
+        for (int o = 0; o < gO; ++o) {
+          const int cc = op.out.c0 + g0 + 8 * o;
+          int slot = 0;
+          if (g.has_dxd) tcc_tma3(dst + slot++ * g.raw_g + o * box, &maps.g[0], l0, cc, n, bar);
+          if (g.has_bn) tcc_tma3(dst + slot++ * g.raw_g + o * box, &maps.g[1], l0, cc, n, bar);
+          if (g.need_x) tcc_tma3(dst + slot * g.raw_g + o * box, &maps.g[2], l0, cc, n, bar);
+        }
+        const uint32_t dx = dst + g.ng * g.raw_g;
+        for (int o = 0; o < xO; ++o) {
+          int cv;
+          const int vi = resolve_view(op, x0 + 8 * o, cv);
+          tcc_tma3(dx + o * box, &maps.x[vi], l0, op.in[vi].c0 + cv, n, bar);
+        }
+        if (++rs == g.raw_stages) { rs = 0; rph ^= 1; }
+      }
+    }
+  } else if (warp >= 4) {
+    const int xw = warp - 4;
+    const int li = lane & 7, lp = lane >> 3;
+    const int QO = g.S / (4 * g.QI);
+    const int items_g = gO * QO, items = (gO + xO) * QO;
+    const bool sig = op.out_act == SEIST_OUT_SIGMOID;
+    const bool elem = op.p_elem > 0.f;
+    const bool want_db = op.dbias != nullptr && (g.split_g || blockIdx.y == 0);
+    const int g_lo = g.g_is_a ? g.part_a : g.part_b, x_lo = g.g_is_a ? g.part_b : g.part_a;
+    int rs = 0, ps = 0;
+    uint32_t rph = 0, pph = 0;
+    for (int tile = blockIdx.x; tile < total && !*abort_s; tile += gridDim.x) {
+      const int n = tile / tiles_per_n;
+      const int l0 = (tile - n * tiles_per_n) * g.S;
+      const float pfaf = path_factor(op, seed, n) * alpha_factor(op, seed, n);
+      if (!tcc_wait(s32(&raw_full[rs]), rph, abort_s)) break;
+      if (!tcc_wait(s32(&p_empty[ps]), pph ^ 1, abort_s)) break;
+      const float* raw = reinterpret_cast<const float*>(raw_s + (size_t)rs * g.raw_stage);
+      unsigned char* pst = p_s + (size_t)ps * g.p_stage;
+      for (int it = xw; it < items; it += TCW_XF_WARPS) {
+        const bool is_g = it < items_g;
+        const int o = (is_g ? it : it - items_g) / QO, qg = (is_g ? it : it - items_g) % QO;
+        const int c = 8 * o + li;
+        if (is_g) {
+          const float4 k = tg_s[c];
+          const bool live = c < gC;
+          float dbs = 0.f;
+#pragma unroll
+          for (int h = 0; h < 2; ++h) {
+            if (h >= g.QI / 4) break;
+            const int q = qg * g.QI + ((li + lp + 4 * h) & (g.QI - 1));
+            const int l = l0 + 4 * q;
+            const int ro = c * g.S + 4 * q;
+            float4 dxd = make_float4(0.f, 0.f, 0.f, 0.f), du = dxd, x = dxd;
+            int slot = 0;
+            if (g.has_dxd) dxd = *reinterpret_cast<const float4*>(raw + slot++ * (g.raw_g >> 2) + ro);
+            if (g.has_bn) du = *reinterpret_cast<const float4*>(raw + slot++ * (g.raw_g >> 2) + ro);
+            if (g.need_x) x = *reinterpret_cast<const float4*>(raw + slot * (g.raw_g >> 2) + ro);
+            float4 v;
+            v.x = tc_out_grad(dxd.x, du.x, x.x, k.x, k.y, k.z, sig, pfaf);
+            v.y = tc_out_grad(dxd.y, du.y, x.y, k.x, k.y, k.z, sig, pfaf);
+            v.z = tc_out_grad(dxd.z, du.z, x.z, k.x, k.y, k.z, sig, pfaf);
+            v.w = tc_out_grad(dxd.w, du.w, x.w, k.x, k.y, k.z, sig, pfaf);
+            if (elem && live && l < L) v = mul4(v, keep4(op.p_elem, seed, op.seed_elem, ((uint64_t)n * op.Cout + g0 + c) * (uint64_t)L + l));
+            if (!live || l >= L) v = make_float4(0.f, 0.f, 0.f, 0.f);
+            dbs += (v.x + v.y) + (v.z + v.w);
+            float4 hi, lo;
+            tcc_split(v.x, hi.x, lo.x);
+            tcc_split(v.y, hi.y, lo.y);
+            tcc_split(v.z, hi.z, lo.z);
+            tcc_split(v.w, hi.w, lo.w);
+            unsigned char* dst = pst + (g.g_is_a ? 0 : 2 * g.part_a) + ((size_t)q * g.g_pitch + c) * 16;
+            *reinterpret_cast<float4*>(dst) = hi;
+            *reinterpret_cast<float4*>(dst + g_lo) = lo;
+          }
+          if (want_db) {
+            dbs += __shfl_xor_sync(0xffffffffu, dbs, 8);
+            dbs += __shfl_xor_sync(0xffffffffu, dbs, 16);
+            if (lp == 0 && live) atomicAdd(&db_s[c], dbs);
+          }
+        } else {
+          const float4 k = tx_s[c];
+          const bool live = c < xC, gl = k.z != 0.f;
+          const float* rx = raw + g.ng * (g.raw_g >> 2);
+#pragma unroll
+          for (int h = 0; h < 2; ++h) {
+            if (h >= g.QI / 4) break;
+            const int q = qg * g.QI + ((li + lp + 4 * h) & (g.QI - 1));
+            const int l = l0 + 4 * q;
+            const float4 r = *reinterpret_cast<const float4*>(rx + c * g.S + 4 * q);
+            float4 v = make_float4(0.f, 0.f, 0.f, 0.f);
+            if (live && l < L) {
+              v.x = tc_conv_input(r.x, k.x, k.y, gl);
+              v.y = tc_conv_input(r.y, k.x, k.y, gl);
+              v.z = tc_conv_input(r.z, k.x, k.y, gl);
+              v.w = tc_conv_input(r.w, k.x, k.y, gl);
+            }
+            float4 hi, lo;
+            tcc_split(v.x, hi.x, lo.x);
+            tcc_split(v.y, hi.y, lo.y);
+            tcc_split(v.z, hi.z, lo.z);
+            tcc_split(v.w, hi.w, lo.w);
+            unsigned char* dst = pst + (g.g_is_a ? 2 * g.part_a : 0) + ((size_t)q * g.x_pitch + c) * 16;
+            *reinterpret_cast<float4*>(dst) = hi;
+            *reinterpret_cast<float4*>(dst + x_lo) = lo;
+          }
+        }
+      }
+      asm volatile("fence.proxy.async.shared::cta;" ::: "memory");
+      __syncwarp();
+      if (lane == 0) {
+        tcc_arrive(s32(&p_full[ps]));
+        tcc_arrive(s32(&raw_empty[rs]));
+      }
+      if (++rs == g.raw_stages) { rs = 0; rph ^= 1; }
+      if (++ps == g.p_stages) { ps = 0; pph ^= 1; }
+    }
+  } else {
+    const uint32_t pitch_a = (uint32_t)(g.part_a / (g.S / 4)), pitch_b = (uint32_t)(g.part_b / (g.S / 4));
+    const int ksteps = g.S >> 3;
+    float acc[MT][NB / 2];
+#pragma unroll
+    for (int m = 0; m < MT; ++m)
+#pragma unroll
+      for (int e = 0; e < NB / 2; ++e) acc[m][e] = 0.f;
+    bool run = true;
+    int ps = 0, prev = -1;
+    uint32_t pph = 0;
+    for (int tile = blockIdx.x; tile < total; tile += gridDim.x) {
+      run = run && tcc_wait(s32(&p_full[ps]), pph, abort_s);
+      const uint32_t a_hi = s32(p_s + (size_t)ps * g.p_stage), a_lo = a_hi + (uint32_t)g.part_a;
+      const uint32_t b_hi = a_hi + 2u * (uint32_t)g.part_a, b_lo = b_hi + (uint32_t)g.part_b;
+      asm volatile("wgmma.fence.sync.aligned;" ::: "memory");
+      for (int j = 0; j < ksteps; ++j) {
+        const uint32_t aoff = (uint32_t)(2 * j) * pitch_a, boff = (uint32_t)(2 * j) * pitch_b;
+        const uint64_t bh = tcc_desc(b_hi + boff, pitch_b, 128), bl = tcc_desc(b_lo + boff, pitch_b, 128);
+#pragma unroll
+        for (int m = 0; m < MT; ++m) {
+          const uint64_t ah = tcc_desc(a_hi + aoff + m * 1024, pitch_a, 128), al = tcc_desc(a_lo + aoff + m * 1024, pitch_a, 128);
+          tcc_mma<NB>(acc[m], ah, bh, 1u);
+          tcc_mma<NB>(acc[m], al, bh, 1u);
+          tcc_mma<NB>(acc[m], ah, bl, 1u);
+        }
+      }
+      asm volatile("wgmma.commit_group.sync.aligned;" ::: "memory");
+      asm volatile("wgmma.wait_group.sync.aligned 1;" ::: "memory");
+      if (prev >= 0) {
+        __syncwarp();
+        if (lane == 0) tcc_arrive(s32(&p_empty[prev]));
+      }
+      prev = ps;
+      if (++ps == g.p_stages) { ps = 0; pph ^= 1; }
+    }
+    asm volatile("wgmma.wait_group.sync.aligned 0;" ::: "memory");
+#pragma unroll
+    for (int m = 0; m < MT; ++m) tcc_keep(acc[m]);
+    if (run && !*abort_s) {
+      const int wq = warp;
+      const int mC = g.g_is_a ? gC : xC, nC = g.g_is_a ? xC : gC;
+#pragma unroll
+      for (int m = 0; m < MT; ++m) {
+#pragma unroll
+        for (int e = 0; e < NB / 2; ++e) {
+          const int row = 64 * m + 16 * wq + (lane >> 2) + 8 * ((e >> 1) & 1);
+          const int col = 8 * (e >> 2) + 2 * (lane & 3) + (e & 1);
+          if (row < mC && col < nC) {
+            const int co = g0 + (g.g_is_a ? row : col), ci = x0 + (g.g_is_a ? col : row);
+            atomicAdd(&op.dW[(size_t)co * op.Cin + ci], acc[m][e]);
+          }
+        }
+      }
+    }
+  }
+
+  __syncthreads();
+  if (op.dbias != nullptr && (g.split_g || blockIdx.y == 0) && !*abort_s)
+    for (int c = tid; c < gC; c += TCW_NT) atomicAdd(&op.dbias[g0 + c], db_s[c]);
+  if (tid == 0 && *abort_s) atomicExch(&g_tcw_err_dev, 1);
+}
+
+bool tcwgrad_eligible(const SeistOp& op) {
+  if (op.k != 1 || op.stride != 1 || op.groups != 1 || op.pool > 1 || op.up_src_L > 0) return false;
+  if (op.L_in != op.L_out || (op.L_out & 3)) return false;
+  if (op.Cin > 256 || op.Cout > 256 || (op.Cin < op.Cout ? op.Cin : op.Cout) > 128) return false;
+  if (op.dW == nullptr) return false;
+  const bool has_bn = op.out.bn >= 0 && op.out.g != nullptr;
+  if (op.out_dxd == nullptr && !has_bn) return false;
+  auto al = [](const void* p) { return (reinterpret_cast<uintptr_t>(p) & 15) == 0; };
+  if (!al(op.out.x) || (op.out.g && !al(op.out.g)) || (op.out_dxd && !al(op.out_dxd)) || op.out.L != op.L_out) return false;
+  for (int i = 0; i < op.n_in; ++i) {
+    if (op.in[i].L != op.L_in || !al(op.in[i].x)) return false;
+    if (op.n_in > 1 && (op.in[i].C & 7)) return false;
+  }
+  return true;
+}
+
+static bool tcw_geometry(const SeistOp& op, TcwGeom& g, int& NB, int& MT, int& blocks) {
+  g = TcwGeom{};
+  const bool has_bn = op.out.bn >= 0 && op.out.g != nullptr;
+  g.has_dxd = op.out_dxd != nullptr ? 1 : 0;
+  g.has_bn = has_bn ? 1 : 0;
+  g.need_x = (has_bn || op.out_act == SEIST_OUT_SIGMOID) ? 1 : 0;
+  g.ng = g.has_dxd + g.has_bn + g.need_x;
+  const bool g_wide = op.Cout >= op.Cin;
+  const int Cm = g_wide ? op.Cout : op.Cin, Cn = g_wide ? op.Cin : op.Cout;
+  NB = Cn <= 16 ? 16 : (Cn <= 32 ? 32 : (Cn <= 64 ? 64 : 128));
+  const int mt_regs = NB == 128 ? 2 : 3;
+  g.g_is_a = g_wide ? 1 : 0;
+  g.split_g = g_wide ? 1 : 0;
+  const int n8 = (Cn + 7) & ~7;
+  for (int mt = (Cm + 63) / 64 < mt_regs ? (Cm + 63) / 64 : mt_regs; mt >= 1; --mt) {
+    const int blk = 64 * mt;
+    const int m8 = ((Cm < blk ? Cm : blk) + 7) & ~7;
+    const int gC8 = g_wide ? m8 : n8, xC8 = g_wide ? n8 : m8;
+    const int S_opts[3] = {64, 32, 16};
+    for (int si = 0; si < 3; ++si) {
+      const int S = S_opts[si];
+      const int raw_stage = S * 4 * (g.ng * gC8 + xC8);
+      const int part_a = (S / 4) * m8 * 16, part_b = (S / 4) * n8 * 16;
+      const int p_stage = 2 * (part_a + part_b);
+      const int fixed = TCW_PANEL_SLACK + 16 * (gC8 + xC8) + 4 * gC8 + 4 * TCW_MAX_STAGES * 8 + 64 + 128 + 64;
+      int ps = TCW_MAX_P_STAGES, st = 0;
+      for (; ps >= 2; --ps) {
+        const int avail = TCW_SMEM_BUDGET - fixed - ps * p_stage;
+        st = avail > 0 ? avail / raw_stage : 0;
+        if (st >= 2) break;
+      }
+      if (ps < 2) continue;
+      if (st > TCW_MAX_STAGES) st = TCW_MAX_STAGES;
+      MT = mt;
+      blocks = (Cm + blk - 1) / blk;
+      g.S = S;
+      g.QI = S == 16 ? 4 : 8;
+      g.blk = blk;
+      g.g0 = 0; g.x0 = 0;
+      g.gC = g_wide ? blk : op.Cout;
+      g.xC = g_wide ? op.Cin : blk;
+      g.g_pitch = gC8;
+      g.x_pitch = xC8;
+      g.raw_stages = st;
+      g.raw_stage = raw_stage;
+      g.raw_g = gC8 * S * 4;
+      g.part_a = part_a;
+      g.part_b = part_b;
+      g.p_stage = p_stage;
+      g.p_stages = ps;
+      int off = 0;
+      g.off_raw = off; off += st * raw_stage;
+      g.off_p = off; off += ps * p_stage + TCW_PANEL_SLACK;
+      g.off_tab_g = off; off += 16 * gC8;
+      g.off_tab_x = off; off += 16 * xC8;
+      g.off_db = off; off += 4 * gC8;
+      off = (off + 15) & ~15;
+      g.off_bar = off; off += 4 * TCW_MAX_STAGES * 8 + 64;
+      g.smem_bytes = off + 128;
+      return true;
+    }
+  }
+  return false;
+}
+
+template <int NB, int MT>
+static int tcw_go(const SeistOp& op, const TcwGeom& g, const TcwMaps& maps, dim3 grid, cudaStream_t s) {
+  static bool attr_set[64] = {false};
+  int dev = 0;
+  cudaGetDevice(&dev);
+  if (!attr_set[dev & 63]) {
+    cudaError_t e = cudaFuncSetAttribute(tcwgrad_kernel<NB, MT>, cudaFuncAttributeMaxDynamicSharedMemorySize, TCW_SMEM_BUDGET + 1024);
+    if (e != cudaSuccess) { set_error(cudaGetErrorString(e)); return (int)e; }
+    attr_set[dev & 63] = true;
+  }
+  tcwgrad_kernel<NB, MT><<<grid, TCW_NT, g.smem_bytes, s>>>(op, g, maps);
+  return 0;
+}
+
+int launch_tcwgrad(const SeistOp& op, cudaStream_t s, int ctas) {
+  TcwGeom g;
+  int NB = 0, MT = 0, blocks = 1;
+  if (!tcw_geometry(op, g, NB, MT, blocks)) { set_error("tcwgrad: no shared-memory configuration"); return -2; }
+  TcwMaps maps;
+  std::memset(&maps, 0, sizeof(maps));
+  int rc = 0;
+  if (g.has_dxd) rc = tcc_make_map(&maps.g[0], op.out_dxd, op.out.L, op.out.Ct, op.N, g.S);
+  if (!rc && g.has_bn) rc = tcc_make_map(&maps.g[1], op.out.g, op.out.L, op.out.Ct, op.N, g.S);
+  if (!rc && g.need_x) rc = tcc_make_map(&maps.g[2], op.out.x, op.out.L, op.out.Ct, op.N, g.S);
+  for (int i = 0; i < op.n_in && !rc; ++i) rc = tcc_make_map(&maps.x[i], op.in[i].x, op.in[i].L, op.in[i].Ct, op.N, g.S);
+  if (rc) return rc;
+  const long tiles = (long)op.N * ((op.L_out + g.S - 1) / g.S);
+  long gx = (ctas + blocks - 1) / blocks;
+  if (gx > tiles) gx = tiles;
+  if (gx < 1) gx = 1;
+  const dim3 grid((unsigned)gx, (unsigned)blocks);
+  if (NB == 16) rc = MT == 1 ? tcw_go<16, 1>(op, g, maps, grid, s) : MT == 2 ? tcw_go<16, 2>(op, g, maps, grid, s) : tcw_go<16, 3>(op, g, maps, grid, s);
+  else if (NB == 32) rc = MT == 1 ? tcw_go<32, 1>(op, g, maps, grid, s) : MT == 2 ? tcw_go<32, 2>(op, g, maps, grid, s) : tcw_go<32, 3>(op, g, maps, grid, s);
+  else if (NB == 64) rc = MT == 1 ? tcw_go<64, 1>(op, g, maps, grid, s) : MT == 2 ? tcw_go<64, 2>(op, g, maps, grid, s) : tcw_go<64, 3>(op, g, maps, grid, s);
+  else rc = MT == 1 ? tcw_go<128, 1>(op, g, maps, grid, s) : tcw_go<128, 2>(op, g, maps, grid, s);
+  if (rc) return rc;
+  note_launch();
+  return check_launch("tcwgrad");
+}
+
+int tcwgrad_error_flag() {
+  int v = 0;
+  cudaMemcpyFromSymbol(&v, g_tcw_err_dev, sizeof(int));
+  return v;
+}
+
+}
```

Measured after the change: 9476, median of 6. 1.02x the previous value.
